# Briimbo/HwBloomRadixJoin

Measured on AMD Instinct MI355X. Metric: probe-tuples/sec, |R|=128M |S|=1024M q=0.01, 1/2/4/8 MI355X; %HBM roofline, higher is better.
Workload: dtype int32

## Files before the change

### hwbloomradixjoin_amd/__init__.py

```python
from __future__ import annotations

import contextlib
import ctypes
import os
from dataclasses import dataclass
from typing import Optional

import numpy as np

__all__ = [
    "BASIC", "BLOCKED", "SECTORIZED", "BloomFilterArgs", "Relation", "Result", "Stats",
    "BPRO", "PRO", "join_materialize_device", "set_materialize", "set_gpus", "BPRH", "BPRHO", "BRJ", "PRH", "PRHO", "RJ", "assert_args", "join_device", "join_device_async", "join_wait", "join_wait_all", "set_async_timing", "generate_device", "generate_device_range",
    "generate_host", "nonunique_threshold", "create_relation_nonunique",
    "create_relation_nonunique_from_pk", "create_relation_fk_from_pk", "create_relation_zipf",
    "rand_stream", "reference_relations", "create_relation_zipf_device",
    "export_filter", "hash_crc", "hash_crapwow", "lib", "LIB_PATH", "shard_range", "write_relation",
]

PKG_DIR = os.path.dirname(os.path.abspath(__file__))
LIB_PATH = os.environ.get("HWBRJ_LIB") or os.path.join(PKG_DIR, "libhwbrj.so")
CLI_PATH = os.path.join(PKG_DIR, "mchashjoins")

BASIC, BLOCKED, SECTORIZED = 0, 1, 2
_VARIANTS = {"basic": BASIC, "blocked": BLOCKED, "sectorized": SECTORIZED}


class _Tuple(ctypes.Structure):
    _fields_ = [("key", ctypes.c_int32), ("payload", ctypes.c_int32)]


class _Relation(ctypes.Structure):
    _fields_ = [("tuples", ctypes.POINTER(_Tuple)), ("num_tuples", ctypes.c_uint64)]


class _Result(ctypes.Structure):
    _fields_ = [("totalresults", ctypes.c_int64), ("resultlist", ctypes.c_void_p),
                ("nthreads", ctypes.c_int)]


class _BloomArgs(ctypes.Structure):
    _fields_ = [("variant", ctypes.c_int), ("m", ctypes.c_uint64), ("k", ctypes.c_uint64),
                ("B", ctypes.c_uint64)]


class _Stats(ctypes.Structure):
    _fields_ = [("filtered", ctypes.c_uint64), ("matches", ctypes.c_int64), ("mode", ctypes.c_int),
                ("format", ctypes.c_int), ("partitions", ctypes.c_uint32),
                ("subparts", ctypes.c_uint32), ("slice_segments", ctypes.c_uint32)] + [
                    (n, ctypes.c_double) for n in (
                        "ms_total", "ms_r_scatter", "ms_r_index", "ms_build", "ms_s_scatter",
                        "ms_s_index", "ms_probe", "ms_surv", "ms_join", "ms_join_probe")] + [
                    ("join_keys", ctypes.c_int), ("unstaged_items", ctypes.c_uint32),
                    ("join_key_bits", ctypes.c_uint32)]

JOIN_KEYS_32, JOIN_KEYS_PACKED, JOIN_KEYS_MIXED = 0, 1, 2


_LIB = None


def lib() -> ctypes.CDLL:
    global _LIB
    if _LIB is None:
        if not os.path.exists(LIB_PATH):
            raise ImportError(f"{LIB_PATH} is missing: run `python -c 'import __graft_entry__ as g; "
                              "g.build()'` (the MI355X HIP library is required; there is no CPU "
                              "fallback)")
        try:
            import torch
        except ImportError:
            pass
        L = ctypes.CDLL(LIB_PATH)
        L.BPRO.restype = ctypes.POINTER(_Result)
        L.BPRO.argtypes = [ctypes.POINTER(_Relation), ctypes.POINTER(_Relation), ctypes.c_int,
                           ctypes.POINTER(_BloomArgs)]
        L.PRO.restype = ctypes.POINTER(_Result)
        L.PRO.argtypes = [ctypes.POINTER(_Relation), ctypes.POINTER(_Relation), ctypes.c_int]
        for nm in ("BPRH", "BPRHO", "BRJ"):
            getattr(L, nm).restype = ctypes.POINTER(_Result)
            getattr(L, nm).argtypes = L.BPRO.argtypes
        for nm in ("PRH", "PRHO", "RJ"):
            getattr(L, nm).restype = ctypes.POINTER(_Result)
            getattr(L, nm).argtypes = L.PRO.argtypes
        L.assert_args.argtypes = [ctypes.POINTER(_BloomArgs)]
        L.hwbrj_join_device.restype = ctypes.c_int
        L.hwbrj_join_device_async.restype = ctypes.c_int
        L.hwbrj_join_device_async.argtypes = [ctypes.c_void_p, ctypes.c_uint64, ctypes.c_void_p,
                                              ctypes.c_uint64, ctypes.c_void_p, ctypes.c_void_p]
        L.hwbrj_join_device_algo.restype = ctypes.c_int
        L.hwbrj_join_device_algo.argtypes = [ctypes.c_void_p, ctypes.c_uint64, ctypes.c_void_p,
                                             ctypes.c_uint64, ctypes.POINTER(_BloomArgs),
                                             ctypes.c_int, ctypes.c_void_p, ctypes.POINTER(_Stats)]
        L.hwbrj_join_wait.restype = ctypes.c_int
        L.hwbrj_join_wait.argtypes = [ctypes.c_void_p]
        L.hwbrj_set_async_timing.restype = ctypes.c_int
        L.hwbrj_set_async_timing.argtypes = [ctypes.c_int]
        L.hwbrj_join_wait_all.restype = ctypes.c_int
        L.hwbrj_join_wait_all.argtypes = [ctypes.c_void_p, ctypes.c_int, ctypes.POINTER(ctypes.c_int)]
        L.hwbrj_join_device.argtypes = [ctypes.c_void_p, ctypes.c_uint64, ctypes.c_void_p,
                                        ctypes.c_uint64, ctypes.POINTER(_BloomArgs),
                                        ctypes.c_void_p, ctypes.POINTER(_Stats)]
        L.hwbrj_join_materialize_device.restype = ctypes.c_int
        L.hwbrj_join_materialize_device.argtypes = [
            ctypes.c_void_p, ctypes.c_uint64, ctypes.c_void_p, ctypes.c_uint64,
            ctypes.POINTER(_BloomArgs), ctypes.c_void_p, ctypes.c_uint64,
            ctypes.POINTER(ctypes.c_uint64), ctypes.c_void_p, ctypes.POINTER(_Stats),
            ctypes.POINTER(ctypes.c_double)]
        L.hwbrj_set_materialize.restype = None
        L.hwbrj_set_materialize.argtypes = [ctypes.c_int]
        L.hwbrj_set_gpus.restype = ctypes.c_int
        L.hwbrj_set_gpus.argtypes = [ctypes.c_int]
        L.hwbrj_generate_device.restype = ctypes.c_int
        L.hwbrj_generate_device.argtypes = [ctypes.c_void_p, ctypes.c_uint64, ctypes.c_uint32,
                                            ctypes.c_uint64, ctypes.c_uint64, ctypes.c_double,
                                            ctypes.c_uint64, ctypes.c_void_p]
        L.hwbrj_generate_device_range.restype = ctypes.c_int
        L.hwbrj_generate_device_range.argtypes = [ctypes.c_void_p, ctypes.c_uint64, ctypes.c_uint64,
                                                  ctypes.c_uint64, ctypes.c_uint32, ctypes.c_uint64,
                                                  ctypes.c_uint64, ctypes.c_double, ctypes.c_uint64,
                                                  ctypes.c_void_p]
        L.hwbrj_generate_host.restype = ctypes.c_int
        L.hwbrj_generate_host.argtypes = [ctypes.c_void_p, ctypes.c_uint64, ctypes.c_uint32,
                                          ctypes.c_uint64, ctypes.c_uint64, ctypes.c_double,
                                          ctypes.c_uint64, ctypes.c_int]
        L.hwbrj_nonunique_threshold.restype = ctypes.c_uint64
        L.hwbrj_nonunique_threshold.argtypes = [ctypes.c_uint64, ctypes.c_double, ctypes.c_int]
        L.hwbrj_create_relation_nonunique.restype = ctypes.c_int
        L.hwbrj_create_relation_nonunique.argtypes = [ctypes.c_void_p, ctypes.c_uint64,
                                                      ctypes.c_int64, ctypes.c_uint32]
        for fn in (L.hwbrj_create_relation_nonunique_from_pk, L.hwbrj_create_relation_fk_from_pk):
            fn.restype = ctypes.c_int
            fn.argtypes = [ctypes.c_void_p, ctypes.c_uint64, ctypes.c_void_p, ctypes.c_uint64,
                           ctypes.c_int64, ctypes.c_double, ctypes.c_uint32]
        L.hwbrj_create_relation_zipf.restype = ctypes.c_int
        L.hwbrj_create_relation_zipf.argtypes = [ctypes.c_void_p, ctypes.c_uint64, ctypes.c_uint64,
                                                 ctypes.c_double, ctypes.c_uint32, ctypes.c_int]
        L.hwbrj_create_relation_zipf_device.restype = ctypes.c_int
        L.hwbrj_create_relation_zipf_device.argtypes = [
            ctypes.c_void_p, ctypes.c_uint64, ctypes.c_uint64, ctypes.c_double, ctypes.c_uint32,
            ctypes.c_double, ctypes.c_int, ctypes.c_void_p]
        L.hwbrj_rand_stream.restype = ctypes.c_int
        L.hwbrj_rand_stream.argtypes = [ctypes.c_uint32, ctypes.c_void_p, ctypes.c_uint64]
        L.hwbrj_write_relation.restype = ctypes.c_int
        L.hwbrj_write_relation.argtypes = [ctypes.POINTER(_Relation), ctypes.c_char_p]
        L.hwbrj_write_result_relation.restype = ctypes.c_int
        L.hwbrj_write_result_relation.argtypes = [ctypes.c_void_p, ctypes.c_char_p]
        L.hwbrj_export_filter.restype = ctypes.c_int
        L.hwbrj_export_filter.argtypes = [ctypes.c_void_p, ctypes.c_uint64]
        L.hwbrj_hash_crc.restype = ctypes.c_uint32
        L.hwbrj_hash_crc.argtypes = [ctypes.c_uint32, ctypes.c_int32]
        L.hwbrj_hash_crapwow.restype = ctypes.c_uint32
        L.hwbrj_hash_crapwow.argtypes = [ctypes.c_uint32, ctypes.c_int32]
        L.hwbrj_device_count.restype = ctypes.c_int
        L.hwbrj_set_device.restype = ctypes.c_int
        L.hwbrj_set_device.argtypes = [ctypes.c_int]
        L.hwbrj_last_error.restype = ctypes.c_char_p
        L.hwbrj_version.restype = ctypes.c_char_p
        L.hwbrj_set_test_hook.restype = ctypes.c_int
        L.hwbrj_set_test_hook.argtypes = [ctypes.c_int, ctypes.c_int64]
        L.hwbrj_tsc_hz.restype = ctypes.c_uint64
        L.hwbrj_copy_bandwidth.restype = ctypes.c_int
        L.hwbrj_copy_bandwidth.argtypes = [ctypes.c_uint64, ctypes.c_int, ctypes.POINTER(ctypes.c_double)]
        L.hwbrj_release.restype = None
        _LIB = L
    return _LIB


def _err(code: int, what: str):
    if code != 0:
        raise RuntimeError(f"{what} failed ({code}): {lib().hwbrj_last_error().decode()}")


@dataclass
class BloomFilterArgs:
    variant: int = BASIC
    m: int = 256 << 20
    k: int = 8
    B: int = 1024

    @classmethod
    def from_flag(cls, b: str, m: int, k: int, B: int = 1024) -> Optional["BloomFilterArgs"]:
        if b == "no":
            return None
        return cls(_VARIANTS.get(b, BASIC), m, k, B)

    def _c(self) -> _BloomArgs:
        return _BloomArgs(int(self.variant), int(self.m), int(self.k), int(self.B))


@dataclass
class Result:
    totalresults: int
    nthreads: int
    pairs: Optional[np.ndarray] = None


class _TupleBuffer(ctypes.Structure):
    pass


_TupleBuffer._fields_ = [("tuples", ctypes.POINTER(_Tuple)), ("next", ctypes.POINTER(_TupleBuffer))]


class _ChainedTupleBuffer(ctypes.Structure):
    _fields_ = [("buf", ctypes.POINTER(_TupleBuffer)), ("readcursor", ctypes.POINTER(_TupleBuffer)),
                ("writecursor", ctypes.POINTER(_TupleBuffer)), ("writepos", ctypes.c_uint32),
                ("readpos", ctypes.c_uint32), ("readlen", ctypes.c_uint32),
                ("numbufs", ctypes.c_uint32)]


class _ThreadResult(ctypes.Structure):
    _fields_ = [("nresults", ctypes.c_int64), ("results", ctypes.c_void_p),
                ("threadid", ctypes.c_uint32)]


_CB_TUPLES = 1024 * 1024


def _take_result(r) -> Result:
    libc = ctypes.CDLL(None)
    res = r.contents
    pairs = None
    if res.resultlist:
        tl = ctypes.cast(res.resultlist, ctypes.POINTER(_ThreadResult))
        parts = []
        for t in range(res.nthreads):
            cb = ctypes.cast(tl[t].results, ctypes.POINTER(_ChainedTupleBuffer)).contents
            n, b, first = tl[t].nresults, cb.buf, True
            while b and n > 0:
                take = min(n, cb.writepos if first else _CB_TUPLES)
                a = np.ctypeslib.as_array(ctypes.cast(b.contents.tuples, ctypes.POINTER(ctypes.c_int32)),
                                          shape=(take * 2,))
                parts.append(a.reshape(-1, 2).copy())
                n -= take
                b, first = b.contents.next, False
            addr = ctypes.cast(cb.buf, ctypes.c_void_p).value
            while addr:
                b = ctypes.cast(addr, ctypes.POINTER(_TupleBuffer)).contents
                nxt = ctypes.cast(b.next, ctypes.c_void_p).value
                libc.free(ctypes.cast(b.tuples, ctypes.c_void_p))
                libc.free(ctypes.c_void_p(addr))
                addr = nxt
            libc.free(ctypes.c_void_p(tl[t].results))
        libc.free(ctypes.cast(res.resultlist, ctypes.c_void_p))
        pairs = np.concatenate(parts) if parts else np.empty((0, 2), dtype=np.int32)
    out = Result(res.totalresults, res.nthreads, pairs)
    libc.free(r)
    return out


HOOK_JOIN_SPLIT, HOOK_PJ_FAIL_RANK, HOOK_BCAST_NONROOT, HOOK_PJ_PLAN_DIV, HOOK_PJ_ASYNC_FAIL = 1, 2, 3, 4, 5
_HOOK_OFF = {HOOK_JOIN_SPLIT: 0, HOOK_PJ_FAIL_RANK: -1, HOOK_BCAST_NONROOT: 0, HOOK_PJ_PLAN_DIV: 0,
             HOOK_PJ_ASYNC_FAIL: 0}


def version() -> str:
    return lib().hwbrj_version().decode()


def set_test_hook(hook: int, value: int) -> None:
    _err(lib().hwbrj_set_test_hook(hook, int(value)), "hwbrj_set_test_hook")


@contextlib.contextmanager
def hooked(hook: int, value: int):
    set_test_hook(hook, value)
    try:
        yield
    finally:
        set_test_hook(hook, _HOOK_OFF[hook])


def set_gpus(gpus: int) -> None:
    _err(lib().hwbrj_set_gpus(int(gpus)), "hwbrj_set_gpus")


def set_materialize(on: bool) -> None:
    lib().hwbrj_set_materialize(1 if on else 0)


@dataclass
class Stats:
    filtered: int
    matches: int
    mode: int
    format: int
    partitions: int
    subparts: int
    slice_segments: int
    ms_total: float
    ms_r_scatter: float
    ms_r_index: float
    ms_build: float
    ms_s_scatter: float
    ms_s_index: float
    ms_probe: float
    ms_surv: float
    ms_join: float
    ms_join_probe: float
    join_keys: int = 0
    unstaged_items: int = 0
    join_key_bits: int = 32


class Relation:

    def __init__(self, tuples: np.ndarray):
        t = np.ascontiguousarray(tuples, dtype=np.int32)
        if t.ndim != 2 or t.shape[1] != 2:
            raise ValueError("tuples must have shape (N, 2): key, payload")
        self.tuples = t
        self._c = _Relation(t.ctypes.data_as(ctypes.POINTER(_Tuple)), t.shape[0])

    @property
    def num_tuples(self) -> int:
        return self.tuples.shape[0]


def write_relation(rel: "Relation | np.ndarray", filename: str) -> None:
    r = rel if isinstance(rel, Relation) else Relation(rel)
    _err(lib().hwbrj_write_relation(ctypes.byref(r._c), os.fsencode(filename)), "hwbrj_write_relation")


def assert_args(args: BloomFilterArgs) -> bool:
    m, B = int(args.m), int(args.B)
    if m & (m - 1):
        return False
    if args.variant != BASIC and (B <= 0 or B & (B - 1) or m % B):
        return False
    return True


def BPRO(relR: Relation, relS: Relation, nthreads: int, args: BloomFilterArgs) -> Result:
    a = args._c()
    return _take_result(lib().BPRO(ctypes.byref(relR._c), ctypes.byref(relS._c), int(nthreads),
                                   ctypes.byref(a)))


def PRO(relR: Relation, relS: Relation, nthreads: int) -> Result:
    return _take_result(lib().PRO(ctypes.byref(relR._c), ctypes.byref(relS._c), int(nthreads)))


def _run(name: str, relR: Relation, relS: Relation, nthreads: int, args=None) -> Result:
    fn = getattr(lib(), name)
    r = (fn(ctypes.byref(relR._c), ctypes.byref(relS._c), int(nthreads), ctypes.byref(args._c()))
         if args is not None else fn(ctypes.byref(relR._c), ctypes.byref(relS._c), int(nthreads)))
    return _take_result(r)


def BPRH(relR, relS, nthreads, args):
    return _run("BPRH", relR, relS, nthreads, args)


def BPRHO(relR, relS, nthreads, args):
    return _run("BPRHO", relR, relS, nthreads, args)


def BRJ(relR, relS, nthreads, args):
    return _run("BRJ", relR, relS, nthreads, args)


def PRH(relR, relS, nthreads):
    return _run("PRH", relR, relS, nthreads)


def PRHO(relR, relS, nthreads):
    return _run("PRHO", relR, relS, nthreads)


def RJ(relR, relS, nthreads):
    return _run("RJ", relR, relS, nthreads)


def _ptr(t) -> int:
    return int(t.data_ptr())


def _check_rel(R, S):
    import torch
    for name, t in (("R", R), ("S", S)):
        if (not t.is_cuda or t.dtype != torch.int32 or t.dim() != 2 or t.shape[1] != 2
                or not t.is_contiguous()):
            raise ValueError(f"{name} must be a contiguous (N, 2) torch.int32 tensor on the GPU")
    if R.device != S.device:
        raise ValueError(f"R is on {R.device} but S is on {S.device}")
    _err(lib().hwbrj_set_device(R.device.index or 0), "hwbrj_set_device")


def join_device_async(R, S, args: Optional[BloomFilterArgs] = None, stream=None) -> None:
    _check_rel(R, S)
    a = args._c() if args is not None else None
    sp = ctypes.c_void_p(stream.cuda_stream) if stream is not None else None
    _err(lib().hwbrj_join_device_async(_ptr(R), R.shape[0], _ptr(S), S.shape[0],
                                       ctypes.byref(a) if a is not None else None, sp),
         "hwbrj_join_device_async")


def join_wait() -> Stats:
    st = _Stats()
    _err(lib().hwbrj_join_wait(ctypes.byref(st)), "hwbrj_join_wait")
    return Stats(**{n: getattr(st, n) for n, _ in _Stats._fields_})


def set_async_timing(on: bool) -> None:
    _err(lib().hwbrj_set_async_timing(1 if on else 0), "hwbrj_set_async_timing")


def join_wait_all(capacity: int = 256) -> list:
    arr = (_Stats * max(1, capacity))()
    n = ctypes.c_int(0)
    _err(lib().hwbrj_join_wait_all(arr, capacity, ctypes.byref(n)), "hwbrj_join_wait_all")
    return [Stats(**{f: getattr(arr[i], f) for f, _ in _Stats._fields_}) for i in range(n.value)]


ALGO_PRO, ALGO_PRH, ALGO_PRHO = 0, 1, 2


def join_device(R, S, args: Optional[BloomFilterArgs] = None, stream=None,
                algorithm: int = ALGO_PRO) -> Stats:
    _check_rel(R, S)
    st = _Stats()
    a = args._c() if args is not None else None
    sp = ctypes.c_void_p(stream.cuda_stream) if stream is not None else None
# ... 142 lines not shown
```

### hwbloomradixjoin_amd/csrc/hwbrj_api.cpp

```cpp
#include <stdio.h>
#include <stdlib.h>
#include <string.h>
#include <x86intrin.h>

#include <algorithm>
#include <chrono>
#include <mutex>
#include <set>
#include <string>
#include <thread>
#include <vector>

#include "hwbrj_engine.h"

namespace hwbrj {

static thread_local std::string g_last_error;
void set_last_error(const std::string& s) { g_last_error = s; }

}

using namespace hwbrj;

extern "C" {

const char* hwbrj_last_error(void) { return g_last_error.c_str(); }
#ifndef HWBRJ_SRC_SHA
#define HWBRJ_SRC_SHA "dev"
#endif
const char* hwbrj_version(void) {
    static const std::string base = [] {
        std::string k = kernel_build_knobs();
        const std::string d = dev_knobs_string();
        if (!d.empty()) k += (k.empty() ? "" : " ") + d;
        return k;
    }();
    static std::mutex            mu;
    static std::set<std::string> interned;
    std::lock_guard<std::mutex>  lk(mu);
    std::string        k = base;
    const TestHooks&   h = test_hooks();
    auto add = [&](const std::string& w) { k += (k.empty() ? "" : " ") + w; };
    if (h.join_split) add("HWBRJ_HOOK_JOIN_SPLIT=" + std::to_string(h.join_split));
    if (h.pj_fail_rank >= 0) add("HWBRJ_HOOK_PJ_FAIL_RANK=" + std::to_string(h.pj_fail_rank));
    if (h.bcast_nonroot) add("HWBRJ_HOOK_BCAST_NONROOT=" + std::to_string(h.bcast_nonroot));
    if (h.pj_plan_div) add("HWBRJ_HOOK_PJ_PLAN_DIV=" + std::to_string(h.pj_plan_div));
    if (h.pj_async_fail) add("HWBRJ_HOOK_PJ_ASYNC_FAIL=" + std::to_string(h.pj_async_fail));
    const std::string v = std::string("hwbloomradixjoin_amd 0.6 (gfx950) src " HWBRJ_SRC_SHA) +
                          (k.empty() ? "" : " knobs: " + k);
    return interned.insert(v).first->c_str();
}

int hwbrj_set_test_hook(int hook, int64_t value) {
    TestHooks& h = test_hooks();
    switch (hook) {
        case HWBRJ_HOOK_JOIN_SPLIT:
            if (value < 0 || value > 0xFFFFFFFFll) break;
            h.join_split = (uint32_t) value;
            return 0;
        case HWBRJ_HOOK_PJ_FAIL_RANK:
            h.pj_fail_rank = (int) value;
            return 0;
        case HWBRJ_HOOK_BCAST_NONROOT:
            if (value < 0 || value > 2) break;
            h.bcast_nonroot = (int) value;
            return 0;
        case HWBRJ_HOOK_PJ_PLAN_DIV:
            if (value < 0 || value > 1000000) break;
            h.pj_plan_div = (int) value;
            return 0;
        case HWBRJ_HOOK_PJ_ASYNC_FAIL:
            if (value < 0 || value > 1) break;
            h.pj_async_fail = (int) value;
            return 0;
        default:
            set_last_error("unknown test hook");
            return 2;
    }
    set_last_error("test hook value out of range");
    return 2;
}

int hwbrj_device_count(void) {
    int n = 0;
    if (hipGetDeviceCount(&n) != hipSuccess) return 0;
    return n;
}

int hwbrj_set_device(int device) {
    hipError_t e = hipSetDevice(device);
    if (e != hipSuccess) {
        set_last_error(std::string("hipSetDevice: ") + hipGetErrorString(e));
        return 1;
    }
    return 0;
}

void hwbrj_release(void) {
    Engine* e = engine_for_current_device();
    if (e) e->release();
}

uint64_t hwbrj_tsc_hz(void) {
    static const uint64_t hz = [] {
        const auto     t0 = std::chrono::steady_clock::now();
        const uint64_t c0 = __rdtsc();
        std::this_thread::sleep_for(std::chrono::milliseconds(50));
        const uint64_t c1 = __rdtsc();
        const double   s  = std::chrono::duration<double>(std::chrono::steady_clock::now() - t0).count();
        return (uint64_t) ((double) (c1 - c0) / s);
    }();
    return hz;
}

int hwbrj_copy_bandwidth(uint64_t bytes, int reps, double* gbps) {
    if (!gbps || reps < 1 || bytes < 16 || bytes % 16) {
        set_last_error("hwbrj_copy_bandwidth: bytes must be a positive multiple of 16, reps >= 1");
        return 1;
    }
    void *a = nullptr, *b = nullptr;
    if (hipMalloc(&a, bytes) != hipSuccess || hipMalloc(&b, bytes) != hipSuccess) {
        if (a) (void) hipFree(a);
        set_last_error("hwbrj_copy_bandwidth: hipMalloc failed");
        return 6;
    }
    hipStream_t st = nullptr;
    hipEvent_t  e0 = nullptr, e1 = nullptr;
    int         rc = 0;
    std::vector<float> ms;
    if (hipStreamCreateWithFlags(&st, hipStreamNonBlocking) != hipSuccess || hipEventCreate(&e0) != hipSuccess ||
        hipEventCreate(&e1) != hipSuccess || hipMemsetAsync(a, 1, bytes, st) != hipSuccess) {
        rc = 3;
    } else {
        int dev = 0, cus = 256;
        (void) hipGetDevice(&dev);
        (void) hipDeviceGetAttribute(&cus, hipDeviceAttributeMultiprocessorCount, dev);
        launch_copy_bw(a, b, bytes, cus, st);
        for (int r = 0; r < reps && rc == 0; r++) {
            float t = 0;
            (void) hipEventRecord(e0, st);
            launch_copy_bw(a, b, bytes, cus, st);
            (void) hipEventRecord(e1, st);
            if (hipEventSynchronize(e1) != hipSuccess || hipEventElapsedTime(&t, e0, e1) != hipSuccess) rc = 3;
            ms.push_back(t);
        }
    }
    if (rc == 0) {
        std::sort(ms.begin(), ms.end());
        *gbps = 2.0 * (double) bytes / (ms[ms.size() / 2] * 1e-3) / 1e9;
    } else {
        set_last_error(std::string("hwbrj_copy_bandwidth: ") + hipGetErrorString(hipGetLastError()));
    }
    if (e0) (void) hipEventDestroy(e0);
    if (e1) (void) hipEventDestroy(e1);
    if (st) (void) hipStreamDestroy(st);
    (void) hipFree(a);
    (void) hipFree(b);
    return rc;
}

uint32_t hwbrj_hash_crc(uint32_t seed, int32_t key) { return crc_f_bitwise(seed ^ (uint32_t) key); }
uint32_t hwbrj_hash_crapwow(uint32_t seed, int32_t key) { return crapwow(seed, (uint32_t) key); }

int hwbrj_join_device(const tuple_t* d_R, uint64_t nR, const tuple_t* d_S, uint64_t nS,
                      const bloom_filter_args_t* args, void* stream, hwbrj_stats_t* stats) {
    Engine* e = engine_for_current_device();
    if (!e) return 10;
    return e->run((const uint2*) d_R, nR, (const uint2*) d_S, nS, args, (hipStream_t) stream, stats);
}

int hwbrj_join_device_algo(const tuple_t* d_R, uint64_t nR, const tuple_t* d_S, uint64_t nS,
                           const bloom_filter_args_t* args, int algorithm, void* stream,
                           hwbrj_stats_t* stats) {
    Engine* e = engine_for_current_device();
    if (!e) return 10;
    return e->run((const uint2*) d_R, nR, (const uint2*) d_S, nS, args, (hipStream_t) stream, stats, algorithm);
}

int hwbrj_join_device_async(const tuple_t* d_R, uint64_t nR, const tuple_t* d_S, uint64_t nS,
                            const bloom_filter_args_t* args, void* stream) {
    Engine* e = engine_for_current_device();
    if (!e) return 10;
    return e->run_async((const uint2*) d_R, nR, (const uint2*) d_S, nS, args, (hipStream_t) stream);
}

int hwbrj_join_partitioned(const hwbrj_exchange_t* x, int rank, int world, const tuple_t* d_R,
                           uint64_t nR, uint64_t nR_total, const tuple_t* d_S, uint64_t nS,
                           const bloom_filter_args_t* args, hwbrj_stats_t* stats) {
    if (!x || !x->buffer || !x->alltoall_u64 || !x->alltoallv || !x->allgather) {
        set_last_error("incomplete exchange (hwbrj_exchange_t)");
        return 2;
    }
    Engine* e = engine_for_current_device();
    if (!e) return 10;
    return e->join_partitioned(x, rank, world, (const uint2*) d_R, nR, nR_total, (const uint2*) d_S, nS,
                               args, stats);
}

int hwbrj_join_wait(hwbrj_stats_t* stats) {
    Engine* e = engine_for_current_device();
    if (!e) return 10;
    return e->wait(stats);
}

int hwbrj_set_async_timing(int on) {
    Engine* e = engine_for_current_device();
    if (!e) return 10;
    e->set_async_timing(on != 0);
    return 0;
}

int hwbrj_join_wait_all(hwbrj_stats_t* stats, int capacity, int* n_joins) {
    if (capacity < 0 || (capacity > 0 && !stats)) {
        set_last_error("stats must hold capacity >= 0 entries");
        return 2;
    }
    Engine* e = engine_for_current_device();
    if (!e) return 10;
    return e->wait_all(stats, capacity, n_joins);
}

static int materialize_pairs(Engine* e, const tuple_t* d_R, uint64_t nR, const tuple_t* d_S, uint64_t nS,
                             const bloom_filter_args_t* args, tuple_t* d_out, uint64_t cap, uint64_t* n,
                             hipStream_t stream, hwbrj_stats_t* st, double* ms) {
    int rc = e->run_mat((const uint2*) d_R, nR, (const uint2*) d_S, nS, args, stream,
                        MatReq{(uint2*) d_out, cap}, st);
    if (rc == 0) {
        *n = (uint64_t) st->matches;
        if (ms) *ms = st->ms_total;
        return 0;
    }
    if (rc != kRcMatGlobal) return rc;
    rc = e->run((const uint2*) d_R, nR, (const uint2*) d_S, nS, args, stream, st);
// ... 445 lines not shown
```

### hwbloomradixjoin_amd/csrc/hwbrj_engine.cpp

```cpp
#include "hwbrj_engine.h"

#include <stdio.h>
#include <stdlib.h>
#include <string.h>

#include <algorithm>
#include <mutex>
#include <vector>

namespace hwbrj {

#define HWBRJ_CHECK(expr)                                                                 \
    do {                                                                                  \
        hipError_t e_ = (expr);                                                           \
        if (e_ != hipSuccess) {                                                           \
            set_last_error(std::string(#expr) + ": " + hipGetErrorString(e_));            \
            return 1;                                                                     \
        }                                                                                 \
    } while (0)

bool build_crc_tables(CrcTables* t) {
    uint32_t col[32];
    for (int i = 0; i < 32; i++) col[i] = crc_f_bitwise(1u << i);
    for (int j = 0; j < 8; j++)
// ... 113 lines not shown
            g->B          = (uint32_t) B;
            g->nblocks    = (uint32_t) std::min<uint64_t>(m / B, 0xFFFFFFFFull);
            g->block_span = (uint32_t) ((B / 8) * 8);
        }
        uint64_t F = 0;
        if (a->variant == BASIC) {
            if (k >= 1 && m >= 32 && k * nR <= (1ull << 31)) {
                g->mode = MODE_SLICE_BASIC;
                F       = std::min<uint64_t>(1024, m / 32);
            } else {
                g->mode = MODE_GLOBAL;
            }
        } else {
            if (B >= 8 && m >= 32 && (m / B) <= 0xFFFFFFFFull) {
                g->mode = MODE_SLICE_BLOCK;
                F       = std::min<uint64_t>(std::min<uint64_t>(1024, m / B), m / 32);
                if (dev_knobs().maxf) F = std::min<uint64_t>(F, dev_knobs().maxf);
            } else {
                g->mode = MODE_GLOBAL;
            }
        }
        g->log2F = (g->mode == MODE_GLOBAL) ? kMaxLog2F : ilog2u(F);
        if (g->mode == MODE_SLICE_BLOCK || g->mode == MODE_SLICE_BASIC) {
            g->slice_bits = (uint32_t) (m >> g->log2F);
            g->seg_bits   = std::min(g->slice_bits, kSliceMaxBits);
            g->nseg       = g->slice_bits / g->seg_bits;
            g->seg_words  = std::max<uint32_t>(4, g->seg_bits / 32);
        }
        if (g->mode == MODE_SLICE_BLOCK && ilog2u(B) <= g->log2F) g->format = FMT_PACKED;
        g->s_format = g->format;
        if (g->mode == MODE_SLICE_BLOCK || g->mode == MODE_SLICE_BASIC) g->log2seg = ilog2u(g->seg_bits);
        if (a->variant != BASIC) {
            g->log2B    = ilog2u(B);
            g->log2secw = std::min<uint32_t>(g->log2B, 6);
            g->nsecmask = (uint32_t) (B >> g->log2secw) - 1u;
            if (g->mode == MODE_SLICE_BLOCK) g->lbmask = (g->nblocks >> g->log2F) - 1u;
        }
    }
    const uint64_t F    = 1ull << g->log2F;
    const uint64_t rper = (nR + F - 1) / F;
    uint32_t       l2s  = 0;
    g->sub_shift  = (g->mode == MODE_SLICE_BASIC) ? 0 : g->log2F;
    if (mat && g->sub_shift > 0) {
        l2s = g->log2F >= 15 ? 0 : std::min<uint32_t>(6, 15 - g->log2F);
        while (l2s < 6 && (rper >> l2s) > 4000) l2s++;
    } else if (mat) {
        while (l2s < 6 && (rper >> l2s) > 1536) l2s++;
    } else if (g->sub_shift > 0 && g->log2F + 6 >= 14) {
        l2s = g->log2F >= 14 ? 0 : 14 - g->log2F;
        if (dev_knobs().l2sub && g->log2F + dev_knobs().l2sub >= 14)
            l2s = std::min<uint32_t>(6, dev_knobs().l2sub);
    } else {
        while (l2s < 6 && (rper >> l2s) > 4096) l2s++;
    }
    if (g->sub_shift + l2s == 0) l2s = 1;
    g->log2NSUB   = l2s;
    g->hash_shift = g->sub_shift + g->log2NSUB;
    return true;
}

bool DevBuf::ensure(size_t need) {
    if (need == 0) need = 16;
    if (need <= bytes) return true;
    release();
    if (hipMalloc(&p, need) != hipSuccess) {
        p     = nullptr;
        bytes = 0;
        return false;
    }
    bytes = need;
    return true;
}

void DevBuf::release() {
    if (p) (void) hipFree(p);
    p     = nullptr;
    bytes = 0;
}

const DevKnobs& dev_knobs() {
    static const DevKnobs k = [] {
        DevKnobs d;
#ifdef HWBRJ_DEV_BUILD
        auto u = [](const char* n) -> uint32_t {
            const char* e = getenv(n);
            return e ? (uint32_t) strtoul(e, nullptr, 0) : 0u;
        };
        d.kk1       = getenv("HWBRJ_DEV_KK1") != nullptr;
        d.kk_gather = getenv("HWBRJ_DEV_KK_GATHER") != nullptr;
        d.noxcd     = getenv("HWBRJ_DEV_NOXCD") != nullptr;
        d.dbg       = getenv("HWBRJ_DBG") != nullptr;
        d.maxf      = u("HWBRJ_DEV_MAXF");
        d.scwpc     = u("HWBRJ_DEV_SCWPC");
        if (getenv("HWBRJ_DEV_EVFLAGS")) d.evflags = (int) u("HWBRJ_DEV_EVFLAGS");
        d.l2sub     = u("HWBRJ_DEV_L2SUB");
        d.ovl       = getenv("HWBRJ_DEV_OVL") != nullptr;
        d.rfirst    = getenv("HWBRJ_DEV_RFIRST") != nullptr;
#endif
        return d;
    }();
    return k;
}

std::string dev_knobs_string() {
    const DevKnobs& d = dev_knobs();
    std::string     r;
    auto add = [&](const std::string& w) { r += (r.empty() ? "" : " ") + w; };
    if (d.kk1) add("HWBRJ_DEV_KK1");
    if (d.kk_gather) add("HWBRJ_DEV_KK_GATHER");
    if (d.noxcd) add("HWBRJ_DEV_NOXCD");
    if (d.dbg) add("HWBRJ_DBG");
    if (d.maxf) add("HWBRJ_DEV_MAXF=" + std::to_string(d.maxf));
    if (d.scwpc) add("HWBRJ_DEV_SCWPC=" + std::to_string(d.scwpc));
    if (d.evflags >= 0) add("HWBRJ_DEV_EVFLAGS=" + std::to_string(d.evflags));
    if (d.l2sub) add("HWBRJ_DEV_L2SUB=" + std::to_string(d.l2sub));
    if (d.ovl) add("HWBRJ_DEV_OVL");
    if (d.rfirst) add("HWBRJ_DEV_RFIRST");
    return r;
}

TestHooks& test_hooks() {
    static TestHooks h;
    return h;
}

Engine::Engine(int device) : device_(device) {
    (void) dev_knobs();
    (void) hipSetDevice(device);
    hipDeviceProp_t prop;
    if (hipGetDeviceProperties(&prop, device) == hipSuccess) cus_ = prop.multiProcessorCount;
    (void) hipStreamCreateWithFlags(&own_stream_, hipStreamNonBlocking);
    const unsigned evf = dev_knobs().evflags >= 0 ? (unsigned) dev_knobs().evflags : hipEventDisableSystemFence;
    for (int i = 0; i < 10; i++)
        (void) (i < 8 ? hipEventCreateWithFlags(&ev_[i], evf) : hipEventCreate(&ev_[i]));
    CrcTables t;
    if (!build_crc_tables(&t)) set_last_error("CRC table inversion failed");
    (void) hipMalloc((void**) &d_tabs_, sizeof(CrcTables));
    (void) hipMemcpy(d_tabs_, &t, sizeof(CrcTables), hipMemcpyHostToDevice);
    (void) hipMalloc((void**) &d_plan_, sizeof(GenPlan));
}

Engine::~Engine() { release(); }

void Engine::release() {
    (void) pj_drain();
    pj_q_.clear();
    if (pj_plan_.valid) pj_lost_ = true;
    for (DevBuf* b : {&pjX, &pjRitems, &pjRing}) b->release();
    for (DevBuf* b : {&poolR, &metaR, &usedR, &wgqcR, &wgqeR, &wgqoR, &lstartR, &estartR, &istartR,
                      &listR, &poolS, &metaS, &usedS, &wgqcS, &wgqeS, &wgqoS, &lstartS, &estartS,
                      &istartS, &listS, &slices, &bitmap, &rjoin, &rrun, &surv, &survcnt, &survoff,
                      &dense, &small, &bpos, &colR, &colS, &mtab, &mcount, &jtask, &jparts, &pjList,
                      &pjLstart, &pjSweep, &pjTab, &pjRegion, &pjTot, &pjSoff, &pjIbase, &pjCnt, &pjOff,
                      &pjIstart, &pjJobs, &ppoolR, &ppoolS, &rpay, &survpos, &dense2, &kkcnt, &xcnt_, &pjBsum, &pjBound, &pjWtot, &pjWscan, &pjTab2})
        b->release();
    for (DevBuf& b : xslot_) b.release();
    if (pending_) (void) hipEventSynchronize(ev_[8]);
    ring_drop();
    jring_.release();
    have_filter_ = false;
}

static size_t ring_slot_bytes() { return 128 + join_sum_slots() * join_sum_stride() * 8; }

static uint64_t region_cap(uint64_t n, uint32_t G, uint32_t F) {
    const uint64_t units = (n + 3) / 4;
    const uint64_t per   = ((units + G - 1) / G) * 4;
    return (per + 31) / 32 + F + 1;
}

int Engine::run(const uint2* dR, uint64_t nR, const uint2* dS, uint64_t nS,
                const bloom_filter_args_t* args, hipStream_t stream, hwbrj_stats_t* st, int jkind) {
    const int rc = enqueue(dR, nR, dS, nS, args, stream, dev_knobs().dbg, jkind);
    return rc ? rc : wait(st);
}

int Engine::run_async(const uint2* dR, uint64_t nR, const uint2* dS, uint64_t nS,
                      const bloom_filter_args_t* args, hipStream_t stream, int jkind) {
    phase_ev_    = false;
    const int rc = enqueue(dR, nR, dS, nS, args, stream, false, jkind);
    phase_ev_    = true;
    return rc;
}

hipError_t Engine::mark(int i, hipStream_t stream) {
    return phase_ev_ ? hipEventRecord(ev_[i], stream) : hipSuccess;
}

int Engine::reserve(const uint2* dR, uint64_t nR, const uint2* dS, uint64_t nS,
                    const bloom_filter_args_t* args, int jkind) {
    alloc_only_  = true;
    const int rc = enqueue(dR, nR, dS, nS, args, nullptr, false, jkind);
    alloc_only_  = false;
    last_nj_     = 0;
    return rc;
}

int Engine::run_mat(const uint2* dR, uint64_t nR, const uint2* dS, uint64_t nS,
                    const bloom_filter_args_t* args, hipStream_t stream, const MatReq& mat,
                    hwbrj_stats_t* st) {
    const int rc = enqueue(dR, nR, dS, nS, args, stream, false, 0, &mat);
    return rc ? rc : wait(st);
}

int Engine::enqueue(const uint2* dR, uint64_t nR, const uint2* dS, uint64_t nS,
                    const bloom_filter_args_t* args, hipStream_t stream, bool dbg, int jkind,
                    const MatReq* mat) {
    if (jkind < 0 || jkind > 2) {
        set_last_error("unknown per-partition join algorithm");
        return 2;
    }
    HWBRJ_CHECK(hipSetDevice(device_));
    Geometry    g;
    std::string err;
    if (!plan_geometry(args, nR, &g, &err, mat != nullptr)) {
        set_last_error(err);
        return 2;
    }
    if (mat && g.mode == MODE_GLOBAL) {
        set_last_error("global-bitmap mode: materialized by the side pass");
        return kRcMatGlobal;
    }
    const bool kk1 = dev_knobs().kk1;
    if (!mat && g.mode == MODE_SLICE_BASIC && (g.k > 1 || kk1) && (uint64_t) g.k * nR <= (1ull << 31) &&
        !dev_knobs().kk_gather) {
        if (!stream) stream = own_stream_;
        if (pending_ && stream != pending_stream_) HWBRJ_CHECK(hipStreamWaitEvent(stream, ev_[8], 0));
        return enqueue_basic_kk(dR, nR, dS, nS, g, stream, jkind);
    }
    if (!stream) stream = own_stream_;
    if (pending_ && stream != pending_stream_) HWBRJ_CHECK(hipStreamWaitEvent(stream, ev_[8], 0));
    const uint32_t F = 1u << g.log2F, NSUB = 1u << g.log2NSUB, NJ = F * NSUB;
    const bool     slice_mode = g.mode == MODE_SLICE_BLOCK || g.mode == MODE_SLICE_BASIC;
    const uint32_t nseg       = slice_mode ? g.nseg : 1;
    const uint32_t CH         = probe_chunks_per_item();
    const size_t   sc_lds     = mat ? scatter_pay_lds_bytes(g.log2F) : scatter_lds_bytes(g.log2F);
    uint32_t       sc_wpc     = (uint32_t) std::max<size_t>(1, std::min<size_t>(2, 163840 / sc_lds));
    if (dev_knobs().scwpc)
        sc_wpc = std::max(1u, std::min(sc_wpc, dev_knobs().scwpc));
    const uint32_t G          = (uint32_t) cus_ * sc_wpc;
    const bool     basic_kk = g.mode == MODE_SLICE_BASIC && g.k > 1;
    const uint64_t nRk      = basic_kk ? (uint64_t) g.k * nR : 0;
    const bool bcast = bcast_ && comm_ && slice_mode && !basic_kk;
    auto pre = [&](int rc) -> int {
        if (!bcast || alloc_only_) return rc;
        return rccl_agree_status(comm_, comm_world_, comm_rank_, rc, stream, &agree_);
    };
    const uint64_t capR = region_cap(nR, G, F), capS = region_cap(std::max(nS, nRk), G, F);
    const uint64_t LR = (uint64_t) G * capR, LS = (uint64_t) G * capS;
    const uint64_t items_max = (LS / CH + F + 1) * nseg;
    if (G > 512) {
        set_last_error("more than 512 scatter workgroups (k_plan row groups)");
        return pre(3);
    }
    if (LS > (1ull << 27) || LR > (1ull << 27) || capS >= (1u << 22) || capR >= (1u << 22)) {
        set_last_error("relation too large for 27-bit chunk ids (|S| or |R| > ~4.2e9 tuples per GPU)");
        return pre(3);
    }
    if (mat && (capS >= (1u << 21) || capR >= (1u << 21))) {
        set_last_error("relation too large for the materializing scatter's 22-bit half indices");
        return pre(3);
    }
    const uint64_t GF = (uint64_t) G * F;
    bool ok = true;
    ok &= poolR.ensure(LR * 128) && metaR.ensure(LR * 2) && listR.ensure(LR * 4);
    ok &= usedR.ensure(G * 4) && wgqcR.ensure(GF * 4) && wgqeR.ensure(GF * 4) && wgqoR.ensure(GF * 4);
    ok &= lstartR.ensure((F + 1) * 4) && estartR.ensure((F + 1) * 8) && istartR.ensure((F + 1) * 4);
    ok &= poolS.ensure(LS * 128) && metaS.ensure(LS * 2) && listS.ensure(LS * 4);
    ok &= usedS.ensure(G * 4) && wgqcS.ensure(GF * 4) && wgqeS.ensure(GF * 4) && wgqoS.ensure(GF * 4);
    ok &= lstartS.ensure((F + 1) * 4) && estartS.ensure((F + 1) * 8) && istartS.ensure((F + 1) * 4);
    const uint64_t BSW = build_chunks_per_sweep(), SLOT = build_sweep_slot();
    const uint64_t sweeps_max = LR / BSW + F + 1;
    ok &= rjoin.ensure(sweeps_max * SLOT * 4) && rrun.ensure(2 * sweeps_max * NSUB * 4);
    ok &= surv.ensure(nseg * LS * 128) && survcnt.ensure(items_max * NSUB * 4) &&
          survoff.ensure(items_max * NSUB * 4);
    ok &= jring_.ensure(kJoinRing * ring_slot_bytes()) && colR.ensure(F * 12) && colS.ensure(F * 12);
    const bool jnew = jparts.bytes < (size_t) (2 * NJ + 1) * 4 || NJ != last_nj_;
    last_nj_ = NJ;
    ok &= jtask.ensure((size_t) join_extra_tasks() * 8) && jparts.ensure((size_t) (2 * NJ + 1) * 4);
    if (slice_mode) ok &= slices.ensure((uint64_t) F * nseg * g.seg_words * 4);
    if (g.mode == MODE_GLOBAL) ok &= bitmap.ensure(((g.m + 31) / 32) * 4) && dense.ensure(nS * 4);
    if (basic_kk) ok &= bpos.ensure(nRk * 4);
    if (mat) {
        ok &= ppoolR.ensure(LR * 128) && ppoolS.ensure(LS * 128) && rpay.ensure(sweeps_max * SLOT * 4) &&
              survpos.ensure(nseg * LS * 128);
    }
    if (!ok) {
        set_last_error("hipMalloc failed (device memory)");
        return pre(4);
    }
    if (alloc_only_) return 0;
    if (const int rc = pre(0)) return rc;
    uint32_t  rslot      = 0;
    bool      rtimed     = false;
    char*     sm         = (char*) ring_take(&rslot);
    if (!sm) return 1;
    uint64_t* d_result   = (uint64_t*) sm;
    uint64_t* d_dcount   = (uint64_t*) sm + 1;
    uint64_t* d_filtered = (uint64_t*) sm + 2;

    if (jnew) HWBRJ_CHECK(hipMemsetAsync(jparts.p, 0, jparts.bytes, stream));
    if (g.mode == MODE_GLOBAL) HWBRJ_CHECK(hipMemsetAsync(bitmap.p, 0, bitmap.bytes, stream));

    ScatterParams sp{};
    sp.tabs = d_tabs_;
    sp.g    = g;
    sp.zero_small = (uint32_t*) sm;
    sp.zero_word  = jparts.as<uint32_t>() + 2 * NJ;

    auto s_pass = [&](hipStream_t st, bool marks, hipEvent_t* tev = nullptr) -> int {
        ScatterParams ss = sp;
        ss.zero_small    = nullptr;
        ss.zero_word     = nullptr;
        if (g.mode == MODE_GLOBAL) {
            launch_probe_global(dS, nS, g, d_tabs_, bitmap.as<uint32_t>(), dense.as<uint32_t>(),
                                d_dcount, st);
            ss.src   = dense.p;
            ss.n     = nS;
            ss.n_dev = d_dcount;
        } else {
            ss.src   = dS;
            ss.n     = nS;
            ss.n_dev = nullptr;
        }
        ss.pool       = poolS.as<uint32_t>();
        ss.meta       = metaS.as<uint32_t>();
        ss.wg_used    = usedS.as<uint32_t>();
        ss.wgq_chunks = wgqcS.as<uint32_t>();
        ss.wgq_elems  = wgqeS.as<uint32_t>();
        ss.cap        = capS;
        if (dbg) {
            if (!dbgS.ensure((size_t) G * 64)) {
                set_last_error("hipMalloc failed (device memory)");
                return 4;
            }
            HWBRJ_CHECK(hipMemsetAsync(dbgS.p, 0, dbgS.bytes, st));
            ss.dbg = dbgS.as<uint64_t>();
        }
        ss.ppool = mat ? ppoolS.as<uint32_t>() : nullptr;
        if (tev) HWBRJ_CHECK(hipEventRecord(tev[0], st));
        launch_scatter(ss, g.mode == MODE_GLOBAL ? SRC_CODES : SRC_TUPLES, SIDE_S, G, st);
        if (tev) HWBRJ_CHECK(hipEventRecord(tev[1], st));
        if (marks) HWBRJ_CHECK(mark(4, st));
        launch_plan(wgqcS.as<uint32_t>(), wgqeS.as<uint32_t>(), G, g.log2F, wgqoS.as<uint32_t>(),
                    colS.as<uint32_t>() + 2 * F, colS.as<uint64_t>(), st);
        launch_list_fill(metaS.as<uint32_t>(), usedS.as<uint32_t>(), capS, g.log2F, wgqoS.as<uint32_t>(),
                         colS.as<uint32_t>() + 2 * F, colS.as<uint64_t>(), CH, nseg, lstartS.as<uint32_t>(),
                         estartS.as<uint64_t>(), istartS.as<uint32_t>(), listS.as<uint32_t>(), G, st);
        if (marks) HWBRJ_CHECK(mark(5, st));
        return 0;
    };
    HWBRJ_CHECK(mark(0, stream));
    const bool ovl = (dev_knobs().ovl || (HWBRJ_OVL_ASYNC && !phase_ev_)) && g.mode != MODE_GLOBAL && !basic_kk &&
                     !mat && !bcast;
    if (ovl) {
        if (!ovl_stream_) {
            HWBRJ_CHECK(hipStreamCreateWithFlags(&ovl_stream_, hipStreamNonBlocking));
            HWBRJ_CHECK(hipEventCreateWithFlags(&ovl_ev_[0], hipEventDisableTiming));
            HWBRJ_CHECK(hipEventCreateWithFlags(&ovl_ev_[1], hipEventDisableTiming));
        }
        HWBRJ_CHECK(hipEventRecord(ovl_ev_[0], stream));
        HWBRJ_CHECK(hipStreamWaitEvent(ovl_stream_, ovl_ev_[0], 0));
        hipEvent_t* tev = nullptr;
        if (async_timing_) {
            for (int i = 0; i < 2; i++)
                if (!tev_[rslot][i]) HWBRJ_CHECK(hipEventCreateWithFlags(&tev_[rslot][i], hipEventDisableSystemFence));
            tev = tev_[rslot];
        }
        rtimed = tev != nullptr;
        if (const int rc = s_pass(ovl_stream_, false, tev)) return rc;
        HWBRJ_CHECK(hipEventRecord(ovl_ev_[1], ovl_stream_));
    }
    const bool s_first = !ovl && !dev_knobs().rfirst && g.mode != MODE_GLOBAL && !basic_kk;
    if (s_first)
        if (const int rc = s_pass(stream, true)) return rc;
    if (g.mode == MODE_GLOBAL)
        launch_build_global(dR, nR, g, d_tabs_, bitmap.as<uint32_t>(), stream);
    sp.src        = dR;
    sp.n          = nR;
    sp.n_dev      = nullptr;
    sp.pool       = poolR.as<uint32_t>();
    sp.ppool      = mat ? ppoolR.as<uint32_t>() : nullptr;
    sp.meta       = metaR.as<uint32_t>();
    sp.wg_used    = usedR.as<uint32_t>();
    sp.wgq_chunks = wgqcR.as<uint32_t>();
    sp.wgq_elems  = wgqeR.as<uint32_t>();
    sp.cap        = capR;
    launch_scatter(sp, SRC_TUPLES, SIDE_R, G, stream);
    HWBRJ_CHECK(mark(1, stream));
    launch_plan(wgqcR.as<uint32_t>(), wgqeR.as<uint32_t>(), G, g.log2F, wgqoR.as<uint32_t>(),
                colR.as<uint32_t>() + 2 * F, colR.as<uint64_t>(), stream);
    launch_list_fill(metaR.as<uint32_t>(), usedR.as<uint32_t>(), capR, g.log2F, wgqoR.as<uint32_t>(),
                     colR.as<uint32_t>() + 2 * F, colR.as<uint64_t>(), (uint32_t) BSW, 1, lstartR.as<uint32_t>(),
                     estartR.as<uint64_t>(), istartR.as<uint32_t>(), listR.as<uint32_t>(), G, stream);
    HWBRJ_CHECK(mark(2, stream));
    sp.ppool      = nullptr;
    sp.zero_small = nullptr;
    sp.zero_word  = nullptr;
    BuildParams bp{};
    bp.g          = g;
    bp.tabs       = d_tabs_;
    bp.pool       = poolR.as<uint32_t>();
    bp.list       = listR.as<uint32_t>();
    bp.list_start = lstartR.as<uint32_t>();
    bp.elem_start = estartR.as<uint64_t>();
    bp.slices     = slice_mode ? slices.as<uint32_t>() : nullptr;
    bp.sweep_start = istartR.as<uint32_t>();
    bp.out_codes   = rjoin.as<uint32_t>();
    bp.run_cnt     = rrun.as<uint32_t>();
    bp.run_off     = rrun.as<uint32_t>() + sweeps_max * NSUB;
    bp.ppool       = mat ? ppoolR.as<uint32_t>() : nullptr;
    bp.out_pay     = mat ? rpay.as<uint32_t>() : nullptr;
    const bool     pack3 = !mat && join_pack3(g) && pack3_hint_;
    const uint32_t kbits = pack3 ? join_key_bits(g) : 0u;
    bp.kbits       = kbits;
    const int nonroot_hook = bcast && comm_world_ == 1 ? test_hooks().bcast_nonroot : 0;
    bp.no_slices = bcast && (comm_rank_ != 0 || nonroot_hook) ? 1u : 0u;
    if (nonroot_hook == 2) HWBRJ_CHECK(hipMemsetAsync(slices.p, 0, slices.bytes, stream));
    launch_build(bp, F, stream);
    if (bcast) {
        const int rc = rccl_broadcast(comm_, slices.p, (size_t) F * nseg * g.seg_words * 4, 0, stream);
        if (rc) {
            (void) hipEventRecord(ev_[8], stream);
            pending_        = true;
            pending_stream_ = stream;
            pending_rc_     = rc;
            pending_err_    = hwbrj_last_error();
            return rc;
        }
    }
    if (basic_kk) {
        launch_bitpos(dR, nR, g, bpos.as<uint32_t>(), stream);
        sp.src        = bpos.p;
        sp.n          = nRk;
        sp.n_dev      = nullptr;
        sp.pool       = poolS.as<uint32_t>();
        sp.meta       = metaS.as<uint32_t>();
        sp.wg_used    = usedS.as<uint32_t>();
        sp.wgq_chunks = wgqcS.as<uint32_t>();
        sp.wgq_elems  = wgqeS.as<uint32_t>();
        sp.cap        = capS;
        launch_scatter(sp, SRC_CODES, SIDE_R, G, stream);
        launch_plan(wgqcS.as<uint32_t>(), wgqeS.as<uint32_t>(), G, g.log2F, wgqoS.as<uint32_t>(),
                    colS.as<uint32_t>() + 2 * F, colS.as<uint64_t>(), stream);
        launch_list_fill(metaS.as<uint32_t>(), usedS.as<uint32_t>(), capS, g.log2F, wgqoS.as<uint32_t>(),
                         colS.as<uint32_t>() + 2 * F, colS.as<uint64_t>(), (uint32_t) BSW, 1,
                         lstartS.as<uint32_t>(), estartS.as<uint64_t>(), istartS.as<uint32_t>(),
                         listS.as<uint32_t>(), G, stream);
        launch_slice_fill(poolS.as<uint32_t>(), listS.as<uint32_t>(), lstartS.as<uint32_t>(), g,
                          slices.as<uint32_t>(), stream);
    }
    HWBRJ_CHECK(mark(3, stream));
    if (ovl) {
        HWBRJ_CHECK(hipStreamWaitEvent(stream, ovl_ev_[1], 0));
        HWBRJ_CHECK(mark(4, stream));
        HWBRJ_CHECK(mark(5, stream));
    } else if (!s_first) {
        if (const int rc = s_pass(stream, true)) return rc;
    }
    ProbeParams pp{};
    pp.g               = g;
    pp.tabs            = d_tabs_;
    pp.pool            = poolS.as<uint32_t>();
    pp.list            = listS.as<uint32_t>();
    pp.list_start      = lstartS.as<uint32_t>();
    pp.item_start      = istartS.as<uint32_t>();
    pp.slices          = slice_mode ? slices.as<uint32_t>() : nullptr;
    pp.surv            = surv.as<uint32_t>();
    pp.surv_seg_stride = LS * 32;
    pp.surv_cnt        = survcnt.as<uint32_t>();
    pp.surv_off        = survoff.as<uint32_t>();
    pp.filtered        = d_filtered;
    pp.job_surv        = jparts.as<uint32_t>() + NJ;
    pp.surv_pos        = mat ? survpos.as<uint32_t>() : nullptr;
    pp.kbits           = kbits;
    pp.fmt_cnt         = mat ? nullptr : (uint32_t*) sm + 10;
    const size_t   pl_lds = probe_lds_bytes(g, nullptr, mat != nullptr);
    const uint32_t PG = (uint32_t) cus_ * (uint32_t) std::max<size_t>(1, std::min<size_t>(2, 163840 / pl_lds));
    const bool dbg_on = dbg;
    if (dbg_on) {
        ok &= dbgP.ensure((size_t) std::max<uint32_t>(PG, F) * 64) && dbgJ.ensure((size_t) std::max<uint64_t>(F, 1024) * 64);
        HWBRJ_CHECK(hipMemsetAsync(dbgP.p, 0, dbgP.bytes, stream));
        HWBRJ_CHECK(hipMemsetAsync(dbgJ.p, 0, dbgJ.bytes, stream));
        pp.dbg = dbgP.as<uint64_t>();
    }
    launch_probe(pp, PG, stream);
    HWBRJ_CHECK(mark(6, stream));
    surv_fused_ = true;
    JoinParams jp{};
    jp.r_codes         = rjoin.as<uint32_t>();
    jp.r_sweep_start   = istartR.as<uint32_t>();
    jp.r_cnt           = rrun.as<uint32_t>();
    jp.r_off           = rrun.as<uint32_t>() + sweeps_max * NSUB;
    jp.slot            = (uint32_t) SLOT;
    jp.surv            = surv.as<uint32_t>();
    jp.surv_cnt        = survcnt.as<uint32_t>();
    jp.surv_off        = survoff.as<uint32_t>();
    jp.item_start      = istartS.as<uint32_t>();
    jp.list_start      = lstartS.as<uint32_t>();
    jp.surv_seg_stride = LS * 32;
    jp.nseg            = nseg;
    jp.CH              = CH;
    jp.log2NSUB        = g.log2NSUB;
    jp.hash_shift      = g.hash_shift;
    jp.bitmap          = (g.sub_shift > 0 && 32 - g.hash_shift <= join_bitmap_log2()) ? 1u : 0u;
    jp.jsum            = (uint64_t*) (sm + 128);
    jp.dbg             = dbg_on ? dbgJ.as<uint64_t>() : nullptr;
    jp.nparts          = jparts.as<uint32_t>();
    jp.extra           = jtask.as<uint2>();
    jp.nextra          = jparts.as<uint32_t>() + 2 * NJ;
    jp.jkind           = (uint32_t) jkind;
    jp.split_surv      = test_hooks().join_split;
    jp.r_kbits         = kbits;
    jp.fmt_cnt         = pp.fmt_cnt;
    jp.timing          = phase_ev_ ? 1u : 0u;
    if (mat) {
        HWBRJ_CHECK(hipMemsetAsync(jparts.as<uint32_t>() + NJ, 0, (size_t) NJ * 4, stream));
        MatJoinParams mp{};
        mp.r_codes         = jp.r_codes;
        mp.r_pay           = rpay.as<uint32_t>();
        mp.r_sweep_start   = jp.r_sweep_start;
        mp.r_cnt           = jp.r_cnt;
        mp.r_off           = jp.r_off;
        mp.slot            = jp.slot;
        mp.surv            = jp.surv;
        mp.surv_pos        = survpos.as<uint32_t>();
        mp.surv_cnt        = jp.surv_cnt;
        mp.surv_off        = jp.surv_off;
        mp.item_start      = jp.item_start;
        mp.list_start      = jp.list_start;
        mp.surv_seg_stride = jp.surv_seg_stride;
        mp.nseg            = nseg;
        mp.CH              = CH;
        mp.log2NSUB        = g.log2NSUB;
        mp.hash_shift      = g.hash_shift;
        mp.bm              = (g.sub_shift > 0 && 32 - g.hash_shift <= 17) ? 1u : 0u;
        mp.s_pay           = ppoolS.as<uint32_t>();
        mp.out             = mat->out;
        mp.cap             = mat->cap;
        mp.count           = (unsigned long long*) d_result;
        launch_join_mat(mp, NJ, stream);
    } else {
        launch_join(jp, NJ, jparts.as<uint32_t>() + NJ, stream);
    }
    HWBRJ_CHECK(hipEventRecord(ev_[8], stream));
    HWBRJ_CHECK(hipGetLastError());
    pending_      = true;
    pending_rc_   = 0;
    pending_args_ = args != nullptr;
    pending_nS_   = nS;
    pending_ev_   = phase_ev_;
    pending_sfirst_ = s_first;
    pending_fmt_    = pp.fmt_cnt != nullptr;
    pending_slots_  = !mat;
    pending_stream_ = stream;
    have_filter_  = args != nullptr;
    last_g_       = g;
    {
        JoinRec r;
        r.slot  = rslot;
        r.args  = args != nullptr;
        r.fmt   = pending_fmt_;
        r.kbits = kbits;
        r.slots = !mat;
        r.timed = rtimed;
        r.nS    = nS;
        r.g     = g;
        ring_push(r);
    }

    if (dbg_on) {
        HWBRJ_CHECK(hipEventSynchronize(ev_[8]));
        std::vector<uint64_t> hp(PG * 8);
        HWBRJ_CHECK(hipMemcpy(hp.data(), dbgP.p, hp.size() * 8, hipMemcpyDeviceToHost));
        double sp_[6] = {0};
        for (uint32_t b = 0; b < PG; b++)
            for (int k = 0; k < 6; k++) sp_[k] += (double) hp[b * 8 + k] / PG;
        std::vector<uint64_t> hs(G * 8);
        HWBRJ_CHECK(hipMemcpy(hs.data(), dbgS.p, hs.size() * 8, hipMemcpyDeviceToHost));
        double ss[6] = {0};
        for (uint32_t b = 0; b < G; b++)
            for (int k = 0; k < 6; k++) ss[k] += (double) hs[b * 8 + k] / G;
        fprintf(stderr, "[dbg] S scatter cyc/WG: hash %.0f load+flush %.0f rank %.0f b1 %.0f write+plan %.0f b2 %.0f\n",
                ss[0], ss[1], ss[2], ss[3], ss[4], ss[5]);
        {
            uint64_t t0 = ~0ull;
            std::vector<double> st(G), en(G);
            for (uint32_t b = 0; b < G; b++) t0 = std::min<uint64_t>(t0, hs[b * 8 + 6]);
            for (uint32_t b = 0; b < G; b++) {
                st[b] = (hs[b * 8 + 6] - t0) / 100.0;
                en[b] = (hs[b * 8 + 7] - t0) / 100.0;
            }
            std::sort(st.begin(), st.end());
            std::sort(en.begin(), en.end());
            fprintf(stderr, "[dbg] S scatter WG start us: max %.1f | end us: min %.1f p10 %.1f p50 %.1f p90 %.1f max %.1f\n",
                    st[G - 1], en[0], en[G / 10], en[G / 2], en[G * 9 / 10], en[G - 1]);
        }
        fprintf(stderr, "[dbg] probe cyc/WG: top %.0f test %.0f b1 %.0f scan+b2 %.0f write %.0f b3+copy %.0f\n",
                sp_[0], sp_[1], sp_[2], sp_[3], sp_[4], sp_[5]);
        {
            std::vector<uint64_t> hj2(1024 * 8);
            HWBRJ_CHECK(hipMemcpy(hj2.data(), dbgJ.p, hj2.size() * 8, hipMemcpyDeviceToHost));
            double sj2[6] = {0};
            const double nwg = (double) F * (1u << g.log2NSUB);
            for (uint32_t b = 0; b < 1024; b++)
                for (int k = 0; k < 6; k++) sj2[k] += (double) hj2[b * 8 + k] / nwg;
            fprintf(stderr, "[dbg] join cyc/WG (wave 0): desc %.0f R+sets %.0f popcnt %.0f surv1 %.0f surv2 %.0f end %.0f\n",
                    sj2[0], sj2[1], sj2[2], sj2[3], sj2[4], sj2[5]);
        }
    }
    return 0;
}

int Engine::enqueue_basic_kk(const uint2* dR, uint64_t nR, const uint2* dS, uint64_t nS,
                             const Geometry& g, hipStream_t stream, int jkind) {
    Geometry    gj;
    std::string err;
    if (!plan_geometry(nullptr, nR, &gj, &err)) {
        set_last_error(err);
        return 2;
    }
    const uint32_t F = 1u << g.log2F, Fj = 1u << gj.log2F, Fm = std::max(F, Fj);
    const uint32_t NSUB = 1u << gj.log2NSUB, NJ = Fj * NSUB;
    const uint32_t nseg = g.nseg, CH = probe_chunks_per_item();
    const uint32_t G    = (uint32_t) cus_;
    const uint64_t nRk  = (uint64_t) g.k * nR;
    const uint64_t Ib   = ((nS / 32 + (uint64_t) G * (Fm + 1)) / CH + Fm + 1) * nseg;
    const uint64_t rw   = ((Ib + G - 1) / G) * CH * 32;
    const uint64_t capR = region_cap(nR, G, Fm);
    const uint64_t capS = std::max(region_cap(std::max(nS, nRk), G, Fm), rw / 32 + Fm + 1);
    const uint64_t LR = (uint64_t) G * capR, LS = (uint64_t) G * capS;
    const uint64_t items_max = (LS / CH + Fm + 1) * nseg;
    if (G > 512 || LS > (1ull << 27) || LR > (1ull << 27) || capS >= (1u << 22) || capR >= (1u << 22)) {
        set_last_error("relation too large for 27-bit chunk ids (|S| or |R| > ~4.2e9 tuples per GPU)");
        return 3;
    }
    const uint64_t GF = (uint64_t) G * Fm;
    bool ok = true;
    ok &= poolR.ensure(LR * 128) && metaR.ensure(LR * 2) && listR.ensure(LR * 4);
    ok &= usedR.ensure(G * 4) && wgqcR.ensure(GF * 4) && wgqeR.ensure(GF * 4) && wgqoR.ensure(GF * 4);
    ok &= lstartR.ensure((Fm + 1) * 4) && estartR.ensure((Fm + 1) * 8) && istartR.ensure((Fm + 1) * 4);
    ok &= poolS.ensure(LS * 128) && metaS.ensure(LS * 2) && listS.ensure(LS * 4);
    ok &= usedS.ensure(G * 4) && wgqcS.ensure(GF * 4) && wgqeS.ensure(GF * 4) && wgqoS.ensure(GF * 4);
    ok &= lstartS.ensure((Fm + 1) * 4) && estartS.ensure((Fm + 1) * 8) && istartS.ensure((Fm + 1) * 4);
    const uint64_t BSW = build_chunks_per_sweep(), SLOT = build_sweep_slot();
    const uint64_t sweeps_max = LR / BSW + Fm + 1;
    ok &= rjoin.ensure(sweeps_max * SLOT * 4) && rrun.ensure(2 * sweeps_max * NSUB * 4);
    ok &= surv.ensure(LS * 128) && survcnt.ensure(items_max * NSUB * 4) && survoff.ensure(items_max * NSUB * 4);
    ok &= jring_.ensure(kJoinRing * ring_slot_bytes()) && colR.ensure(Fm * 12) && colS.ensure(Fm * 12);
    const bool jnew = jparts.bytes < (size_t) (2 * NJ + 1) * 4 || NJ != last_nj_;
    last_nj_ = NJ;
    ok &= jtask.ensure((size_t) join_extra_tasks() * 8) && jparts.ensure((size_t) (2 * NJ + 1) * 4);
    ok &= slices.ensure((uint64_t) F * nseg * g.seg_words * 4) && (g.k <= G || bpos.ensure(nRk * 4));
    const uint32_t NC = (g.k + 64) & ~63u;
    ok &= dense.ensure(G * rw * 4) && dense2.ensure(G * rw * 4) && kkcnt.ensure(NC * 8 + 2 * G * 4);
    if (!ok) {
        set_last_error("hipMalloc failed (device memory)");
        return 4;
    }
    if (alloc_only_) return 0;
    uint32_t  rslot      = 0;
    char*     sm         = (char*) ring_take(&rslot);
    if (!sm) return 1;
    uint64_t* d_filtered = (uint64_t*) sm + 2;
    uint64_t* cnt        = kkcnt.as<uint64_t>();
    uint32_t* wgc[2]     = {(uint32_t*) (cnt + NC), (uint32_t*) (cnt + NC) + G};
    HWBRJ_CHECK(hipMemsetAsync(sm, 0, 64, stream));
    HWBRJ_CHECK(hipMemsetAsync(kkcnt.p, 0, kkcnt.bytes, stream));
    if (jnew) HWBRJ_CHECK(hipMemsetAsync(jparts.p, 0, jparts.bytes, stream));
    HWBRJ_CHECK(hipMemsetAsync(jparts.as<uint32_t>() + 2 * NJ, 0, 4, stream));

    auto side = [&](bool r) {
        ScatterParams sp{};
        sp.tabs       = d_tabs_;
        sp.pool       = (r ? poolR : poolS).as<uint32_t>();
        sp.meta       = (r ? metaR : metaS).as<uint32_t>();
        sp.wg_used    = (r ? usedR : usedS).as<uint32_t>();
        sp.wgq_chunks = (r ? wgqcR : wgqcS).as<uint32_t>();
        sp.wgq_elems  = (r ? wgqeR : wgqeS).as<uint32_t>();
        sp.cap        = r ? capR : capS;
        return sp;
    };
    auto index = [&](bool r, uint32_t log2F, uint32_t ch, uint32_t ns) {
        const uint32_t Fx = 1u << log2F;
        DevBuf& col = r ? colR : colS;
        launch_plan((r ? wgqcR : wgqcS).as<uint32_t>(), (r ? wgqeR : wgqeS).as<uint32_t>(), G, log2F,
                    (r ? wgqoR : wgqoS).as<uint32_t>(), col.as<uint32_t>() + 2 * Fx, col.as<uint64_t>(), stream);
        launch_list_fill((r ? metaR : metaS).as<uint32_t>(), (r ? usedR : usedS).as<uint32_t>(), r ? capR : capS,
                         log2F, (r ? wgqoR : wgqoS).as<uint32_t>(), col.as<uint32_t>() + 2 * Fx, col.as<uint64_t>(),
                         ch, ns, (r ? lstartR : lstartS).as<uint32_t>(), (r ? estartR : estartS).as<uint64_t>(),
                         (r ? istartR : istartS).as<uint32_t>(), (r ? listR : listS).as<uint32_t>(), G, stream);
    };

    HWBRJ_CHECK(mark(0, stream));
    ScatterParams sp = side(true);
    sp.g   = gj;
    sp.src = dR;
    sp.n   = nR;
    launch_scatter(sp, SRC_TUPLES, SIDE_R, G, stream);
    HWBRJ_CHECK(mark(1, stream));
    index(true, gj.log2F, (uint32_t) BSW, 1);
    HWBRJ_CHECK(mark(2, stream));
    BuildParams bp{};
    bp.g           = gj;
    bp.tabs        = d_tabs_;
    bp.pool        = poolR.as<uint32_t>();
    bp.list        = listR.as<uint32_t>();
    bp.list_start  = lstartR.as<uint32_t>();
    bp.elem_start  = estartR.as<uint64_t>();
    bp.sweep_start = istartR.as<uint32_t>();
    bp.out_codes   = rjoin.as<uint32_t>();
    bp.run_cnt     = rrun.as<uint32_t>();
    bp.run_off     = rrun.as<uint32_t>() + sweeps_max * NSUB;
    launch_build(bp, Fj, stream);
    sp = side(false);
    if (g.k <= G) {
        Geometry gp = g;
        gp.mode     = MODE_BASIC_POS;
        sp.g        = gp;
        sp.src      = dR;
        sp.n        = nRk;
        sp.vn       = nR;
        launch_scatter(sp, SRC_TUPLES, SIDE_R, G, stream);
    } else {
        launch_bitpos(dR, nR, g, bpos.as<uint32_t>(), stream);
        sp.g   = g;
        sp.src = bpos.p;
        sp.n   = nRk;
        launch_scatter(sp, SRC_CODES, SIDE_R, G, stream);
    }
    index(false, g.log2F, (uint32_t) BSW, 1);
    launch_slice_fill(poolS.as<uint32_t>(), listS.as<uint32_t>(), lstartS.as<uint32_t>(), g,
                      slices.as<uint32_t>(), stream);
    HWBRJ_CHECK(mark(3, stream));
    sp     = side(false);
    sp.g   = g;
    sp.src = dS;
    sp.n   = nS;
    launch_scatter(sp, SRC_TUPLES, SIDE_S, G, stream);
    HWBRJ_CHECK(mark(4, stream));
    index(false, g.log2F, CH, nseg);
    HWBRJ_CHECK(mark(5, stream));
    const uint32_t PG = G;
    ProbeParams    pb{};
    pb.pool       = poolS.as<uint32_t>();
    pb.list       = listS.as<uint32_t>();
    pb.list_start = lstartS.as<uint32_t>();
    pb.item_start = istartS.as<uint32_t>();
    pb.slices     = slices.as<uint32_t>();
    uint32_t* dz[2] = {dense.as<uint32_t>(), dense2.as<uint32_t>()};
// ... 357 lines not shown
```

### hwbloomradixjoin_amd/csrc/hwbrj_engine.h

```cpp
#pragma once

#include <hip/hip_runtime.h>
#include <stdint.h>

#include <deque>
#include <string>
#include <vector>

#include "../../include/hwbrj.h"
#include "hwbrj_common.h"
#include "hwbrj_kernels.h"

namespace hwbrj {

bool plan_geometry(const bloom_filter_args_t* args, uint64_t nR, Geometry* g, std::string* err,
                   bool mat = false);

struct MatReq {
    uint2*   out;
    uint64_t cap;
};
constexpr int kRcMatGlobal = 11;

struct DevBuf {
// ... 18 lines not shown
    void set_async_timing(bool on) { async_timing_ = on; }
    int  reserve(const uint2* dR, uint64_t nR, const uint2* dS, uint64_t nS,
                 const bloom_filter_args_t* args, int jkind = 0);
    int  export_filter(uint8_t* host_out, uint64_t nbytes);
    int  run_mat(const uint2* dR, uint64_t nR, const uint2* dS, uint64_t nS,
                 const bloom_filter_args_t* args, hipStream_t stream, const MatReq& mat,
                 hwbrj_stats_t* st);
    int  materialize(const uint2* dR, uint64_t nR, const uint2* dS, uint64_t nS, uint2* out,
                     uint64_t cap, uint64_t* n, hipStream_t stream, double* ms);
    int  generate(uint2* d_out, uint64_t n, uint64_t offset, uint64_t count, uint32_t nthreads,
                  uint64_t maxid, uint64_t threshold, double selectivity, uint64_t seed,
                  hipStream_t stream);
    int  join_partitioned(const hwbrj_exchange_t* x, int rank, int world, const uint2* dR,
                          uint64_t nR, uint64_t nR_total, const uint2* dS, uint64_t nS,
                          const bloom_filter_args_t* args, hwbrj_stats_t* st, bool native = false);
    void release();
    int  device() const { return device_; }

    int  comm_init(const uint8_t* unique_id, int world, int rank);
    int  comm_destroy();
    bool has_comm() const { return comm_ != nullptr; }
    int  comm_world() const { return comm_world_; }
    int  comm_rank() const { return comm_rank_; }
    int  join_partitioned_rccl(const uint2* dR, uint64_t nR, uint64_t nR_total, const uint2* dS,
                               uint64_t nS, const bloom_filter_args_t* args, hwbrj_stats_t* st);
    void set_filter_broadcast(bool on) { bcast_ = on; }
    hipStream_t stream() const { return own_stream_; }
    DevBuf*     xslot(int s) { return &xslot_[s]; }
    DevBuf*     xcnt() { return &xcnt_; }
    void*       comm() const { return comm_; }
    hwbrj_exchange_t native_exchange();

    static constexpr int kPjDepth = 8;
    static constexpr int kPjKey   = 10;
    int  join_partitioned_async(const hwbrj_exchange_t* x, int rank, int world, const uint2* dR, uint64_t nR,
                                uint64_t nR_total, const uint2* dS, uint64_t nS, const bloom_filter_args_t* args);
    int  join_partitioned_wait(hwbrj_stats_t* st);
    void pj_async_info(uint64_t* out) const;
    bool pj_make_plan() const { return pj_make_plan_; }
    int  pj_plan_from_sync(int world, int rank, uint64_t nR, uint64_t nR_total, uint64_t nS,
                           const bloom_filter_args_t* args, uint64_t mr, uint64_t mi, uint64_t mw);
    int  pj_drain();

  private:
    struct PjGeom {
        Geometry g{};
        uint32_t F = 0, NSUB = 0, W = 0, QL = 0, q0 = 0, nseg = 1, CH = 0, G = 0, NC = 0, items_max = 0;
        uint64_t BSW = 0, SLOT = 0, capR = 0, capS = 0, LS = 0;
        bool     slice_mode = false;
    };
    struct PjPlan {
        bool     valid = false;
        uint64_t BR = 0, BI = 0, BW = 0;
        uint64_t key[kPjKey] = {};
    };
    struct PjX {
        hwbrj_exchange_t x{};
        bool             native = true;
        int              rank = 0, world = 1;
    };
    struct PjIn {
        PjX                 xc;
        const uint2*        dR = nullptr;
        const uint2*        dS = nullptr;
        uint64_t            nR = 0, nR_total = 0, nS = 0;
        bool                has_args = false;
        bloom_filter_args_t args{};
    };
    struct PjPending {
        PjIn          in;
        PjGeom        G;
        bool          sync = false;
        bool          failed_mode = false;
        int           rc   = 0;
        int           slot = 0;
        hwbrj_stats_t st{};
    };
    bool pj_geom(int world, int rank, uint64_t nR, uint64_t nR_total, uint64_t nS,
                 const bloom_filter_args_t* args, PjGeom* G);
    int  pj_async_alloc(const PjGeom& G, const PjPlan& p, bool all, const PjX& c);
    int  pj_a2a_u64(const PjX& c, const uint64_t* d_send, uint64_t* d_recv, uint64_t n);
    int  pj_max_dev(const PjX& c, uint64_t* d, uint64_t n);
    int  pj_max_host(const PjX& c, uint64_t* h, uint64_t n);
    int  pj_establish_plan(const PjGeom& G, uint64_t mr, uint64_t mi, uint64_t mw, const uint64_t* key);
    int  pj_sync_join(const PjIn& in, hwbrj_stats_t* st);
    PjPlan                pj_plan_;
    PjX                   pj_cur_;
    bloom_filter_args_t   pj_plan_args_{};
    bool                  pj_make_plan_ = false;
    bool                  pj_lost_      = false;
    std::deque<PjPending> pj_q_;
    uint64_t              pj_seq_ = 0, pj_async_ = 0, pj_sync_ = 0, pj_fallbacks_ = 0, pj_plans_ = 0;
    uint64_t              pj_last_flag_ = 0, pj_last_sizes_[3] = {0, 0, 0};
    DevBuf                pjX, pjRitems, pjRing;
    hipEvent_t            pjEv_[2 * kPjDepth] = {};

  private:
    void*        comm_       = nullptr;
    int          comm_world_ = 1, comm_rank_ = 0;
    bool         bcast_      = false;
    DevBuf       xslot_[HWBRJ_PJ_NSLOTS], xcnt_;
    DevBuf       agree_;
    int          device_;
    int          cus_ = 256;
    hipStream_t  own_stream_ = nullptr;
    hipStream_t  ovl_stream_ = nullptr;
    hipEvent_t   ovl_ev_[2]  = {nullptr, nullptr};
    hipEvent_t   ev_[10];
    bool         have_filter_ = false;
    Geometry     last_g_{};
    bool         pending_      = false;
    bool         pending_args_ = false;
    uint64_t     pending_nS_   = 0;
    uint32_t     last_nj_      = 0;
    bool         phase_ev_     = true;
    bool         pending_ev_   = true;
    hipStream_t  pending_stream_ = nullptr;
    bool         pending_sfirst_ = false;
    bool         pending_fmt_    = false;
    bool         pending_slots_  = false;
    bool         pack3_hint_     = true;
    int          pending_rc_     = 0;
    std::string  pending_err_;
    bool         surv_fused_   = false;
    struct JoinRec {
        uint32_t slot = 0;
        bool     args = false, fmt = false, slots = false, timed = false;
        uint32_t kbits = 0;
        uint64_t nS   = 0;
        Geometry g{};
    };
    DevBuf                     jring_;
    std::vector<JoinRec>       jr_;
    std::vector<hwbrj_stats_t> jdone_;
    uint32_t                   jr_next_ = 0;
    hwbrj_stats_t              last_st_{};
    bool                       async_timing_ = false;
    hipEvent_t                 tev_[kJoinRing][2] = {};
    void*        ring_take(uint32_t* slot);
    void         ring_push(const JoinRec& r) { jr_.push_back(r); }
    int          ring_collect();
    void         ring_drop() { jr_.clear(); jdone_.clear(); }
    hipError_t   mark(int i, hipStream_t stream);
    bool         alloc_only_   = false;
    int          enqueue(const uint2* dR, uint64_t nR, const uint2* dS, uint64_t nS,
                         const bloom_filter_args_t* args, hipStream_t stream, bool dbg, int jkind,
                         const MatReq* mat = nullptr);
    int          enqueue_basic_kk(const uint2* dR, uint64_t nR, const uint2* dS, uint64_t nS,
                                  const Geometry& g, hipStream_t stream, int jkind);
    CrcTables*   d_tabs_ = nullptr;
    GenPlan*     d_plan_ = nullptr;
    DevBuf poolR, metaR, usedR, wgqcR, wgqeR, wgqoR, lstartR, estartR, istartR, listR;
    DevBuf poolS, metaS, usedS, wgqcS, wgqeS, wgqoS, lstartS, estartS, istartS, listS;
    DevBuf slices, bitmap, rjoin, rrun, surv, survcnt, survoff, dense, small, dbgP, dbgJ, dbgS;
    DevBuf bpos;
    DevBuf colR, colS;
    DevBuf mtab, mcount;
    DevBuf ppoolR, ppoolS, rpay, survpos;
    DevBuf dense2, kkcnt;
    DevBuf jtask, jparts;
    DevBuf pjList, pjLstart, pjSweep, pjTab, pjRegion, pjTot, pjSoff, pjIbase, pjCnt, pjOff, pjIstart, pjJobs;
    DevBuf pjBsum, pjBound, pjWtot, pjWscan, pjTab2;
};

Engine* engine_for_current_device();
void    set_last_error(const std::string& s);

int rccl_broadcast(void* comm, void* buf, size_t bytes, int root, hipStream_t stream);
int read_join_counts(const void* small, bool slots, hipStream_t stream, uint64_t h[6]);
int rccl_agree_status(void* comm, int world, int rank, int rc, hipStream_t stream, DevBuf* tmp);
class Engine;
int rccl_alltoall_u64_dev(Engine* e, const uint64_t* d_send, uint64_t* d_recv, uint64_t n);
int rccl_allreduce_max_u64(Engine* e, uint64_t* d, uint64_t n);
bool rccl_self_blocks();
uint64_t pj_region_cap(uint64_t n, uint32_t G, uint32_t F);

struct GlibcRand {
    int32_t st[31];
    int     f = 3, r = 0;
    void    seed(uint32_t s);
    int32_t next() {
        st[f]           = (int32_t) ((uint32_t) st[f] + (uint32_t) st[r]);
        const int32_t v = (int32_t) ((uint32_t) st[f] >> 1);
        f               = f == 30 ? 0 : f + 1;
        r               = r == 30 ? 0 : r + 1;
        return v;
    }
};

}
```

### hwbloomradixjoin_amd/csrc/hwbrj_kernels.h

```cpp
#pragma once

#include <hip/hip_runtime.h>

#include <string>
#include <stddef.h>
#include <stdint.h>

#include "hwbrj_common.h"

namespace hwbrj {

enum Source : int { SRC_TUPLES = 0, SRC_CODES = 1 };

struct ScatterParams {
    const void*      src;
    uint64_t         n;
    const uint64_t*  n_dev;
    uint32_t*        pool;
    uint32_t*        ppool;
    uint32_t*        meta;
    uint32_t*        wg_used;
    uint32_t*        wgq_chunks;
    uint32_t*        wgq_elems;
    uint64_t*        dbg;
    uint64_t         cap;
    const uint32_t*  seg_cnt;
    uint64_t         seg_stride;
    uint64_t         vn;
    uint32_t*        zero_small;
    uint32_t*        zero_word;
    Geometry         g;
    const CrcTables* tabs;
};

#ifndef HWBRJ_PACK3
#define HWBRJ_PACK3 1
#endif
#ifndef HWBRJ_PACK18
#define HWBRJ_PACK18 1
#endif
inline bool join_pack3(const Geometry& g) { return HWBRJ_PACK3 != 0 && g.sub_shift > 0 && g.hash_shift >= 8; }
inline uint32_t join_key_bits(const Geometry& g) {
    return !join_pack3(g) ? 0u : (HWBRJ_PACK18 && g.hash_shift == 14) ? 18u : 24u;
}

#ifndef HWBRJ_OVL_ASYNC
#define HWBRJ_OVL_ASYNC 1
#endif
#ifndef HWBRJ_PJ_OVL
#define HWBRJ_PJ_OVL 1
#endif

struct BuildParams {
    Geometry         g;
    const CrcTables* tabs;
    const uint32_t*  pool;
    const uint32_t*  list;
    const uint32_t*  list_start;
    const uint64_t*  elem_start;
    uint32_t*        slices;
    const uint32_t*  sweep_start;
    uint32_t*        out_codes;
    uint32_t*        run_cnt;
    uint32_t*        run_off;
    uint32_t         q_base;
    const uint32_t*  ppool;
    uint32_t*        out_pay;
    uint32_t         no_slices;
    uint32_t         kbits;
};

struct ProbeParams {
    Geometry         g;
    const CrcTables* tabs;
    const uint32_t*  pool;
    const uint32_t*  list;
    const uint32_t*  list_start;
    const uint32_t*  item_start;
    const uint32_t*  slices;
    uint32_t*        surv;
    uint64_t         surv_seg_stride;
    uint32_t*        surv_cnt;
    uint32_t*        surv_off;
    uint64_t*        filtered;
    uint32_t*        job_surv;
    uint32_t         stage_cap;
    uint32_t*        surv_pos;
    uint32_t*        wg_cnt;
    uint64_t*        dbg;
    uint32_t         kbits;
    uint32_t*        fmt_cnt;
};

struct JoinParams {
    const uint32_t* r_codes;
    const uint32_t* r_sweep_start;
    const uint32_t* r_cnt;
    const uint32_t* r_off;
    const uint32_t* surv;
    const uint32_t* surv_cnt;
    const uint32_t* surv_off;
    const uint32_t* item_start;
    const uint32_t* list_start;
    uint64_t        surv_seg_stride;
    uint32_t        nseg, CH, log2NSUB, hash_shift;
    uint32_t        slot;
    uint32_t        bitmap;
    uint64_t*       jsum;
    uint32_t        jobs;
    uint32_t*       nparts;
    uint2*          extra;
    uint32_t*       nextra;
    uint32_t        split_surv;
    uint64_t*       dbg;
    uint32_t        jkind;
    const uint64_t* item_base;
    uint32_t        r_kbits;
    const uint32_t* fmt_cnt;
    uint32_t        timing;
};

struct MatJoinParams {
    const uint32_t* r_codes;
    const uint32_t* r_pay;
    const uint32_t* r_sweep_start;
    const uint32_t* r_cnt;
    const uint32_t* r_off;
    uint32_t        slot;
    const uint32_t* surv;
    const uint32_t* surv_pos;
    const uint32_t* surv_cnt;
    const uint32_t* surv_off;
    const uint32_t* item_start;
    const uint32_t* list_start;
    uint64_t        surv_seg_stride;
    uint32_t        nseg, CH, log2NSUB, hash_shift;
    uint32_t        bm;
    uint32_t        xcd8;
    const uint32_t* s_pay;
    uint2*          out;
    uint64_t        cap;
    unsigned long long* count;
};

void   launch_gen(uint2* out, uint64_t offset, uint64_t count, const GenPlan* d_plan, const Perm& perm,
                  hipStream_t st);
void   launch_zipf(const int32_t* rnd, uint64_t cnt, uint64_t row0, const double* lut,
                   const uint32_t* alphabet, uint32_t size, uint2* out, uint64_t n_above,
                   uint32_t above_base, const Perm& perm, hipStream_t st);
void   launch_build_global(const uint2* R, uint64_t n, const Geometry& g, const CrcTables* tabs,
                           uint32_t* bm, hipStream_t st);
void   launch_probe_global(const uint2* S, uint64_t n, const Geometry& g, const CrcTables* tabs,
                           const uint32_t* bm, uint32_t* out, uint64_t* out_count, hipStream_t st);
void   launch_bitpos(const uint2* R, uint64_t n, const Geometry& g, uint32_t* out, hipStream_t st);
void   launch_slice_fill(const uint32_t* pool, const uint32_t* list, const uint32_t* list_start,
                         const Geometry& g, uint32_t* slices, hipStream_t st);
size_t scatter_lds_bytes(uint32_t log2F);
size_t scatter_pay_lds_bytes(uint32_t log2F);
enum { SIDE_R = 0, SIDE_S = 1 };
void   launch_scatter(const ScatterParams& p, int src, int side, uint32_t grid, hipStream_t st);
void   launch_list_fill(const uint32_t* meta, const uint32_t* wg_used, uint64_t cap,
                        uint32_t log2F, const uint32_t* wgq_off, const uint32_t* colc,
                        const uint64_t* cole, uint32_t CH, uint32_t nseg, uint32_t* list_start,
                        uint64_t* elem_start, uint32_t* item_start, uint32_t* list, uint32_t grid,
                        hipStream_t st);
bool   launch_plan(const uint32_t* wgq_chunks, const uint32_t* wgq_elems, uint32_t G,
                   uint32_t log2F, uint32_t* wgq_off, uint32_t* colc, uint64_t* cole,
                   hipStream_t st);
uint32_t probe_chunks_per_item();
size_t   probe_lds_bytes(const Geometry& g, uint32_t* stage_cap, bool pay = false);
size_t slice_lds_bytes(const Geometry& g);
uint32_t build_chunks_per_sweep();
uint32_t build_sweep_slot();
void   launch_build(const BuildParams& p, uint32_t F, hipStream_t st);
void   launch_probe(const ProbeParams& p, uint32_t grid, hipStream_t st);
size_t probe_bitj_lds_bytes(const Geometry& g);
void   launch_probe_bitj(const ProbeParams& p, uint32_t grid, hipStream_t st);
void   launch_join(const JoinParams& p, uint32_t jobs, uint32_t* job_surv, hipStream_t st);
uint32_t join_extra_tasks();
uint32_t join_sum_slots();
uint32_t join_sum_stride();
uint32_t join_bitmap_log2();
void   launch_join_mat(const MatJoinParams& p, uint32_t jobs, hipStream_t st);
void   launch_mat_build(const uint2* R, uint64_t n, unsigned long long* tab, uint64_t mask,
                        hipStream_t st);
void   launch_mat_probe(const uint2* S, uint64_t n, const uint2* R, const unsigned long long* tab,
                        uint64_t mask, uint2* out, uint64_t cap, unsigned long long* count,
                        const Geometry& g, const uint32_t* slices, const uint32_t* bm,
                        const CrcTables* tabs, hipStream_t st);
void   launch_pj_items(const uint32_t* item_start, const uint32_t* list_start, const uint32_t* cnt,
                       uint32_t items_max, uint32_t F, uint32_t nseg, uint32_t CH, uint64_t seg_words, uint32_t NSUB,
                       uint64_t* region, uint32_t* tot, uint64_t* bsum, uint64_t* sofs, uint64_t* bound,
                       hipStream_t st);
void   launch_pj_recv_scan(const uint32_t* cnt, uint32_t n, uint32_t NSUB, uint32_t* tot, uint64_t* bsum,
                           uint64_t* wscan, hipStream_t st, uint32_t BI = 0, const uint32_t* ritems = nullptr);
void   launch_pj_item_tables(const uint32_t* tab, uint32_t pairs, uint32_t W, const uint32_t* rcnt,
                             const uint64_t* wscan, uint32_t NSUB, uint64_t* ibase, uint32_t* icnt, uint32_t* ioff,
                             uint32_t* jobs, hipStream_t st, uint32_t BI = 0, uint64_t BW = 0);
void   launch_pjx_gather(const uint32_t* pool, const uint32_t* list, const uint32_t* lstart, uint32_t F, uint32_t QL,
                         uint32_t W, uint64_t BR, void* out, uint32_t* ent, int own, void* own_out, uint32_t* own_ent,
                         uint64_t* flag, hipStream_t st);
void   launch_pjx_rtab(const uint64_t* rc, uint32_t W, uint32_t QL, uint32_t NC, uint64_t BR, uint32_t bsw,
                       int64_t* tab, uint32_t* lsO, uint32_t* swO, uint64_t* flag, hipStream_t st);
void   launch_pjx_surv_pack(const uint32_t* surv, const uint64_t* region, const uint32_t* tot, const uint64_t* sofs,
                            const uint32_t* item_start, const uint64_t* bound, const uint32_t* cnt, uint32_t F,
                            uint32_t QL, uint32_t NSUB, uint64_t BI, uint64_t BW, uint32_t* out, uint32_t* out_cnt,
                            int own, uint32_t* own_out, uint32_t* own_cnt, uint64_t* flag, hipStream_t st);
void   launch_pjx_stab(const uint64_t* rc, uint32_t W, uint32_t QL, uint32_t NC, uint64_t BI, uint64_t BW,
                       uint32_t* tab2, uint32_t* istart, uint32_t* ritems, uint64_t* flag, hipStream_t st);
void   launch_pjx_stat(const uint64_t* rc1, const uint64_t* rc2, const uint32_t* ls, const uint32_t* is,
                       const uint64_t* bd, uint32_t W, uint32_t QL, uint32_t NC, const uint64_t* flag, uint64_t* out,
                       hipStream_t st);
struct PjOwn {
    uint32_t  lo = 0, hi = 0;
    int64_t   delta = 0;
    void*     out = nullptr;
    uint32_t* ent = nullptr;
};
void   launch_pj_gather(const uint32_t* pool, const uint32_t* list, uint32_t n, void* out, uint32_t* ent,
                        hipStream_t st, const PjOwn& own = PjOwn{});
void   launch_pj_counts(const uint32_t* starts, const uint64_t* bound, uint32_t W, uint32_t QL, uint32_t NC,
                        uint64_t status, uint64_t extra, uint64_t extra2, uint64_t* out, hipStream_t st);
void   launch_pj_relist(const uint32_t* rent, const int64_t* tab, uint32_t pairs, uint32_t* list,
                        hipStream_t st);
void   launch_pj_surv_pack(const uint32_t* surv, const uint64_t* region, const uint32_t* tot,
                           const uint64_t* soff, uint32_t n, uint32_t* out, hipStream_t st,
                           const PjOwn& own = PjOwn{});
void   launch_export(const uint32_t* slices, const Geometry& g, uint32_t* out, uint64_t nwords,
                     hipStream_t st);
void   launch_copy_bw(const void* src, void* dst, uint64_t bytes, int grid, hipStream_t st);

const char* kernel_build_knobs();

struct DevKnobs {
    bool     kk1 = false;
    bool     kk_gather = false;
    bool     noxcd = false;
    bool     dbg = false;
    uint32_t maxf = 0;
    uint32_t scwpc = 0;
    int      evflags = -1;
    uint32_t l2sub = 0;
    bool     ovl   = false;
    bool     rfirst = false;
};
const DevKnobs& dev_knobs();
std::string dev_knobs_string();

struct TestHooks {
    uint32_t join_split    = 0;
    int      pj_fail_rank  = -1;
    int      bcast_nonroot = 0;
    int      pj_plan_div   = 0;
    int      pj_async_fail = 0;
};
TestHooks& test_hooks();

}
```

### hwbloomradixjoin_amd/csrc/hwbrj_kernels.hip

```cpp
#include <hip/hip_runtime.h>
#include <stdlib.h>

#include <algorithm>
#include <string>
#include <type_traits>

#include "hwbrj_common.h"
#include "hwbrj_kernels.h"

#if !defined(HWBRJ_DEV_BUILD) &&                                                                   \
    (defined(HWBRJ_ABL_NOCRC) || defined(HWBRJ_ABL_NOCRAP) || defined(HWBRJ_ABL_NOSTORE) ||        \
     defined(HWBRJ_ABL_SPLITH) || defined(HWBRJ_ABL_PNOPST) || defined(HWBRJ_ABL_BNOBITS) ||       \
     defined(HWBRJ_ABL_BNOSORT) || defined(HWBRJ_ABL_PNOB1) || defined(HWBRJ_ABL_JNOR) ||          \
     defined(HWBRJ_ABL_JNOS) || defined(HWBRJ_ABL_MJ_EMPTY) || defined(HWBRJ_ABL_MJ_NOLOAD) ||     \
     defined(HWBRJ_ABL_MJ_NOINS) || defined(HWBRJ_ABL_MJ_R) || defined(HWBRJ_ABL_PROBE) ||         \
     defined(HWBRJ_STAMPS))
#error "HWBRJ_ABL_* / HWBRJ_STAMPS give invalid results or perturb timing: dev builds only (-DHWBRJ_DEV_BUILD)"
#endif

namespace hwbrj {

__device__ __forceinline__ void load_tab(uint32_t* dst, const uint32_t* src) {
    for (int i = threadIdx.x; i < 128; i += blockDim.x) dst[i] = src[i];
}
// ... 188 lines not shown
    for (; i < cnt; i += stride) {
        const double r     = ((double) rnd[i]) / 2147483647;
        uint32_t     left  = 0, right = size - 1, pos;
        if (lut[0] >= r) {
            pos = 0;
        } else {
            while (right - left > 1) {
                const uint32_t m = (left + right) / 2;
                if (lut[m] < r) left = m;
                else right = m;
            }
            pos = right;
        }
        const uint64_t row = row0 + i;
        uint32_t       key = alphabet[pos];
        if (n_above) {
            const uint64_t u = perm_apply(perm, row);
            if (u < n_above) key = above_base + (uint32_t) u;
        }
        out[i] = make_uint2(key, (uint32_t) row);
    }
}

void launch_zipf(const int32_t* rnd, uint64_t cnt, uint64_t row0, const double* lut,
                 const uint32_t* alphabet, uint32_t size, uint2* out, uint64_t n_above,
                 uint32_t above_base, const Perm& perm, hipStream_t st) {
    k_zipf<<<8192, 256, 0, st>>>(rnd, cnt, row0, lut, alphabet, size, out, n_above, above_base, perm);
}

__device__ __forceinline__ void global_positions_apply_add(uint32_t key, uint32_t code,
                                                           const Geometry& g, uint32_t* bm) {
    uint64_t base;
    uint32_t size;
    if (g.variant == VAR_BASIC) {
        base = 0;
        size = (uint32_t) g.m;
    } else {
        base = (uint64_t) (code & (g.nblocks - 1u)) * g.block_span;
        size = g.B;
    }
    uint32_t       h  = mod_m(crapwow(kSeed, key), size);
    uint32_t       y  = mod_m(key + kSeed, size);
    const uint32_t s0 = (g.variant == VAR_SECTORIZED) ? h / (g.B < 64u ? g.B : 64u) : 0u;
    for (uint32_t i = 0; i < g.k; i++) {
        const uint32_t pos = (g.variant == VAR_SECTORIZED) ? sectorize(h, s0, i, g.B) : h;
        const uint64_t b   = base + pos;
        atomicOr(bm + (b >> 5), 1u << (uint32_t) (b & 31u));
        h = mod_m(h + y, size);
        y = mod_m(y + i + 1u, size);
    }
}

__device__ __forceinline__ bool global_contains(uint32_t key, uint32_t code, const Geometry& g,
                                                const uint32_t* bm) {
    uint64_t base;
    uint32_t size;
    if (g.variant == VAR_BASIC) {
        base = 0;
        size = (uint32_t) g.m;
    } else {
        base = (uint64_t) (code & (g.nblocks - 1u)) * g.block_span;
        size = g.B;
    }
    uint32_t       h  = mod_m(crapwow(kSeed, key), size);
    uint32_t       y  = mod_m(key + kSeed, size);
    const uint32_t s0 = (g.variant == VAR_SECTORIZED) ? h / (g.B < 64u ? g.B : 64u) : 0u;
    for (uint32_t i = 0; i < g.k; i++) {
        const uint32_t pos = (g.variant == VAR_SECTORIZED) ? sectorize(h, s0, i, g.B) : h;
        const uint64_t b   = base + pos;
        if (!((bm[b >> 5] >> (uint32_t) (b & 31u)) & 1u)) return false;
        h = mod_m(h + y, size);
        y = mod_m(y + i + 1u, size);
    }
    return true;
}

__global__ __launch_bounds__(256) void k_build_global(const uint2* R, uint64_t n, Geometry g,
                                                      const CrcTables* tabs, uint32_t* bm) {
    __shared__ uint32_t fwd[128];
    load_tab(fwd, &tabs->fwd[0][0]);
    __syncthreads();
    uint64_t       i      = blockIdx.x * (uint64_t) blockDim.x + threadIdx.x;
    const uint64_t stride = (uint64_t) gridDim.x * blockDim.x;
    for (; i < n; i += stride) {
        const uint32_t key = R[i].x;
        global_positions_apply_add(key, key_code(fwd, key), g, bm);
    }
}

__global__ __launch_bounds__(1024) void k_probe_global(const uint2* S, uint64_t n, Geometry g,
                                                       const CrcTables* tabs, const uint32_t* bm,
                                                       uint32_t* out, uint64_t* out_count) {
    __shared__ uint32_t fwd[128];
    __shared__ uint32_t wsum[16];
    __shared__ uint64_t bbase;
    load_tab(fwd, &tabs->fwd[0][0]);
    __syncthreads();
    const int wave = threadIdx.x >> 6, lane = threadIdx.x & 63;
    for (uint64_t t0 = (uint64_t) blockIdx.x * 1024; t0 < n; t0 += (uint64_t) gridDim.x * 1024) {
        const uint64_t i    = t0 + threadIdx.x;
        uint32_t       code = 0;
        uint32_t       pass = 0;
        if (i < n) {
            const uint32_t key = S[i].x;
            code               = key_code(fwd, key);
            pass               = global_contains(key, code, g, bm) ? 1u : 0u;
        }
        const uint32_t incl = wave_incl_scan(pass);
        if (lane == 63) wsum[wave] = incl;
        __syncthreads();
        if (threadIdx.x == 0) {
            uint32_t tot = 0;
            for (int w = 0; w < 16; w++) {
                uint32_t c = wsum[w];
                wsum[w]    = tot;
                tot += c;
            }
            bbase = tot ? atomicAdd((unsigned long long*) out_count, (unsigned long long) tot) : 0;
        }
        __syncthreads();
        if (pass) out[bbase + wsum[wave] + incl - 1] = code;
        __syncthreads();
    }
}

__device__ __forceinline__ uint16_t meta16(uint32_t q, uint32_t count) {
    return (uint16_t) (q | ((count - 1u) << 10));
}
#ifndef HWBRJ_SC_T
#define HWBRJ_SC_T 1024
#endif
constexpr int      kScThreads = HWBRJ_SC_T;
constexpr int      kScPlanPer = (1024 + kScThreads - 1) / kScThreads;
constexpr int      kScPayThreads = 1024;
#ifndef HWBRJ_SC_E
#define HWBRJ_SC_E 8
#define HWBRJ_SC_K 2
#endif
#ifndef HWBRJ_SC_PRE
#define HWBRJ_SC_PRE 1
#endif
#ifndef HWBRJ_SC_KEEPY
#define HWBRJ_SC_KEEPY 1
#endif
#ifndef HWBRJ_SC_LAUX
#define HWBRJ_SC_LAUX 2
#endif
#ifndef HWBRJ_SC_SAUX
#define HWBRJ_SC_SAUX 2
#endif
#ifndef HWBRJ_SC_SAUX_R
#define HWBRJ_SC_SAUX_R HWBRJ_SC_SAUX
#endif
constexpr int      kScPre     = HWBRJ_SC_PRE;
constexpr int      kScE       = HWBRJ_SC_E;
constexpr uint32_t kScRound   = kScThreads * kScE;
constexpr int      kScK       = HWBRJ_SC_K;
constexpr uint32_t kCbBits    = 22;
constexpr uint32_t kCbMask    = (1u << kCbBits) - 1u;
constexpr uint32_t kOob       = 0x7FFFFFF0u;

template <int K, bool RIGHT>
__device__ __forceinline__ uint32_t byte_sh2(uint32_t x) {
    static_assert(K >= 0 && K < 4, "byte index");
    uint32_t r;
#define HWBRJ_SDWA(op, sel) asm(op "_sdwa %0, 2, %1 dst_sel:DWORD dst_unused:UNUSED_PAD src0_sel:DWORD src1_sel:" sel : "=v"(r) : "v"(x))
    if (!RIGHT) {
        if (K == 0) HWBRJ_SDWA("v_lshlrev_b32", "BYTE_0");
        if (K == 1) HWBRJ_SDWA("v_lshlrev_b32", "BYTE_1");
        if (K == 2) HWBRJ_SDWA("v_lshlrev_b32", "BYTE_2");
        if (K == 3) HWBRJ_SDWA("v_lshlrev_b32", "BYTE_3");
    } else {
        if (K == 0) HWBRJ_SDWA("v_lshrrev_b32", "BYTE_0");
        if (K == 1) HWBRJ_SDWA("v_lshrrev_b32", "BYTE_1");
        if (K == 2) HWBRJ_SDWA("v_lshrrev_b32", "BYTE_2");
        if (K == 3) HWBRJ_SDWA("v_lshrrev_b32", "BYTE_3");
    }
#undef HWBRJ_SDWA
    return r;
}

__device__ __forceinline__ uint32_t crc_nib(const uint32_t* tab, uint32_t key) {
    const char*    b = (const char*) tab;
    const uint32_t y = key & 0x0F0F0F0Fu, z = key & 0xF0F0F0F0u;
    auto T = [&](uint32_t off) { return *(const uint32_t*) (b + off); };
    const uint32_t t0 = T(byte_sh2<0, false>(y)), t1 = T(byte_sh2<0, true>(z) + 64);
    const uint32_t t2 = T(byte_sh2<1, false>(y) + 128), t3 = T(byte_sh2<1, true>(z) + 192);
    const uint32_t t4 = T(byte_sh2<2, false>(y) + 256), t5 = T(byte_sh2<2, true>(z) + 320);
    const uint32_t t6 = T(byte_sh2<3, false>(y) + 384), t7 = T(byte_sh2<3, true>(z) + 448);
    const uint32_t a = __builtin_amdgcn_bitop3_b32(t0, t1, t2, 0x96);
    const uint32_t c = __builtin_amdgcn_bitop3_b32(t3, t4, t5, 0x96);
    return __builtin_amdgcn_bitop3_b32(a, c, t6 ^ t7, 0x96);
}

template <int SRC, int MODE, int FMT>
__device__ __forceinline__ void sc_word_lds0(uint32_t x, const Geometry& g, const uint32_t* tab,
                                             uint32_t& w, uint32_t& q) {
    const uint32_t F1 = (1u << g.log2F) - 1u;
    if (SRC == SRC_CODES) {
        if (MODE == MODE_BASIC_BITJ) {
            q = basic_bit(bunmix(x), g.bitj, (uint32_t) g.m) & F1;
            w = x;
        } else if (MODE == MODE_CODE_OF_KEY) {
            w = crc_nib(tab, bunmix(x));
            q = w & F1;
        } else {
            w = x;
            q = x & F1;
        }
        return;
    }
    const uint32_t key  = x;
#ifdef HWBRJ_ABL_NOCRC
    const uint32_t code = key * 0x9E3779B1u;
#else
    const uint32_t code = crc_nib(tab, key);
#endif
    if (MODE == MODE_SLICE_BASIC) {
        q = mod_m(crapwow(kSeed, key), (uint32_t) g.m) & F1;
        w = bmix(key);
    } else if (MODE == MODE_SLICE_BLOCK && FMT == FMT_PACKED) {
        q = code & F1;
#ifdef HWBRJ_ABL_NOCRAP
        w = (key & (g.B - 1u)) | ((code >> g.log2F) << g.log2B);
#else
        w = (crapwow(kSeed, key) & (g.B - 1u)) | ((code >> g.log2F) << g.log2B);
#endif
    } else {
        q = code & F1;
        w = code;
    }
}

template <int SRC>
struct ScRaw {
    uint32_t k[SRC == SRC_TUPLES ? kScE : 1];
    uint4    v[SRC == SRC_TUPLES ? 1 : kScE / 4];
    uint32_t jb[SRC == SRC_TUPLES ? kScE : 1];
    uint32_t y[SRC == SRC_TUPLES && HWBRJ_SC_KEEPY ? kScE : 1];
};

template <int SRC, int MODE, int FMT, int SAUX = HWBRJ_SC_SAUX>
__device__ __forceinline__ void scatter_body(const ScatterParams& P) {
    extern __shared__ __attribute__((aligned(16))) uint32_t lds[];
    __shared__ uint32_t crc_tab[128];
    constexpr int NL = SRC == SRC_TUPLES ? kScE / 2 : kScE / 4;
    const uint32_t F     = 1u << P.g.log2F;
    uint32_t*      stage = lds;
    uint32_t*      fill  = stage + F * 32 + 64;
    uint32_t*      ncb   = fill + F + 4;
    uint32_t*      flq   = ncb + 2 * F;
    uint32_t*      misc  = flq + F;
    const int      tid   = threadIdx.x, lane = tid & 63;
    const uint32_t dummy = F * 32 + lane;
    for (uint32_t i = tid; i < F + 1; i += kScThreads) fill[i] = 0;
    uint32_t my_tch[kScPlanPer], my_tel[kScPlanPer];
#pragma unroll
    for (int i = 0; i < kScPlanPer; i++) my_tch[i] = my_tel[i] = 0;
    if (tid < 128) {
        const uint32_t* src = &P.tabs->fwd[0][0];
        uint32_t        v   = src[tid];
        if (tid < 16) {
#pragma unroll
            for (int j = 0; j < 8; j++) v ^= src[j * 16 + ((kSeed >> (4 * j)) & 15u)];
        }
        crc_tab[tid] = v;
    }
    if (tid < 8) misc[tid] = 0;
    if (blockIdx.x == 0 && P.zero_small && tid < 16) P.zero_small[tid] = 0;
    if (blockIdx.x == 0 && P.zero_word && tid == 0) *P.zero_word = 0;

    if (P.dbg && tid == 0) P.dbg[blockIdx.x * 8 + 6] = __builtin_amdgcn_s_memrealtime();
    const uint64_t n     = P.n_dev ? *P.n_dev : P.n;
    const uint64_t units = (n + 3) >> 2;
    const uint64_t G = gridDim.x, wg = blockIdx.x;
    uint64_t       e0  = 4 * (wg * units / G);
    const uint64_t e1r = 4 * ((wg + 1) * units / G);
    const uint64_t e1  = e1r < n ? e1r : n;
    uint32_t       len = __builtin_amdgcn_readfirstlane(e1 > e0 ? (uint32_t) (e1 - e0) : 0u);
    if (SRC == SRC_CODES && P.seg_cnt) {
        e0  = wg * P.seg_stride;
        len = __builtin_amdgcn_readfirstlane(P.seg_cnt[wg]);
    }
    constexpr uint32_t CW = 32u;
    uint32_t* __restrict__ pool = P.pool + wg * P.cap * CW;
    uint16_t* __restrict__ meta = (uint16_t*) P.meta + wg * P.cap;
    constexpr uint32_t EB = SRC == SRC_TUPLES ? 8u : 4u;
    const auto rsrc = buf_rsrc((const uint8_t*) P.src + e0 * EB, len * EB);
    const auto rpool = buf_rsrc(pool, (uint32_t) (P.cap * CW * 4));
    const auto rmeta = buf_rsrc(meta, (uint32_t) (P.cap * 2));
    __syncthreads();

    const uint64_t vn  = MODE == MODE_BASIC_POS && P.vn ? P.vn : 1;
    const uint32_t jb0 = MODE == MODE_BASIC_POS ? (uint32_t) (e0 / vn) : 0u;
    const uint64_t vb  = (uint64_t) (jb0 + 1) * vn;
    auto load_round = [&](uint32_t base, ScRaw<SRC>& R) {
        if (MODE == MODE_BASIC_POS) {
#pragma unroll
            for (int j = 0; j < kScE; j++) {
                const uint32_t i  = base + j * kScThreads + tid;
                const uint64_t ev = e0 + (i < len ? i : 0u);
                uint32_t       jj = jb0;
                for (uint64_t b = vb; ev >= b; b += vn) jj++;
                const uint64_t t = ev - (uint64_t) jj * vn;
                R.k[j]  = len ? ((const uint32_t*) P.src)[2 * t] : 0u;
                R.jb[j] = jj;
            }
        } else if (SRC == SRC_TUPLES && base + kScRound <= len) {
#pragma unroll
            for (int h = 0; h < kScE / 2; h++) {
                const v4u x = __builtin_amdgcn_raw_buffer_load_b128(rsrc, 2 * tid * EB, (base + h * 2 * kScThreads) * EB, HWBRJ_SC_LAUX);
                R.k[2 * h]     = x.x;
                R.k[2 * h + 1] = x.z;
                if (HWBRJ_SC_KEEPY) {
                    R.y[2 * h]     = x.y;
                    R.y[2 * h + 1] = x.w;
                }
            }
        } else if (SRC == SRC_TUPLES) {
#pragma unroll
            for (int j = 0; j < kScE; j++) {
                const uint32_t i = base + (j >> 1) * 2 * kScThreads + 2 * tid + (j & 1);
                R.k[j] = __builtin_amdgcn_raw_buffer_load_b32(rsrc, i < len ? i * EB : kOob, 0, 0);
                if (HWBRJ_SC_KEEPY) R.y[j] = 0;
            }
        } else {
#pragma unroll
            for (int h = 0; h < NL; h++) {
                const uint32_t i = base + h * (4 * kScThreads) + 4 * tid;
                const v4u x = __builtin_amdgcn_raw_buffer_load_b128(rsrc, i < len ? i * EB : kOob, 0, 0);
                R.v[h]      = make_uint4(x.x, x.y, x.z, x.w);
            }
        }
    };
    auto elem = [&](const ScRaw<SRC>& R, uint32_t base, int j, uint32_t& x, uint32_t& idx) {
        if (SRC == SRC_TUPLES) {
            x   = R.k[j];
            idx = MODE == MODE_BASIC_POS ? base + j * kScThreads + tid : base + (j >> 1) * 2 * kScThreads + 2 * tid + (j & 1);
        } else {
            const int h = j >> 2, t = j & 3;
            x   = t == 0 ? R.v[h].x : t == 1 ? R.v[h].y : t == 2 ? R.v[h].z : R.v[h].w;
            idx = base + h * (4 * kScThreads) + 4 * tid + t;
        }
    };
    uint32_t par = 0;
    auto flush_copy = [&]() {
        const uint32_t nf = misc[1 + (par ^ 1u)];
        auto task = [&](uint32_t k) {
            const bool     ok = k < nf * 8;
            const uint32_t qq = flq[ok ? k >> 3 : 0];
            const uint32_t l8 = k & 7;
            const uint32_t cb = ncb[(par ^ 1u) * F + qq] & kCbMask;
            const v4u      v  = *(const v4u*) &stage[qq * 32 + l8 * 4];
#ifdef HWBRJ_ABL_NOSTORE
            if (v.x == 0x12345678u && v.y == 0x9abcdef0u)
#endif
            __builtin_amdgcn_raw_buffer_store_b128(v, rpool, ok ? (cb * 32 + l8 * 4) * 4 : kOob, 0, SAUX);
            __builtin_amdgcn_raw_buffer_store_b16((short) meta16(qq, 32u), rmeta, ok && l8 == 0 ? cb * 2 : kOob, 0, 0);
        };
#pragma unroll
        for (int i = 0; i < kScK; i++) task(tid + i * kScThreads);
        for (uint32_t k = kScK * kScThreads + tid; k < nf * 8; k += kScThreads) task(k);
    };

    uint64_t tph[6] = {0, 0, 0, 0, 0, 0}, tlast = __builtin_amdgcn_s_memtime();
    (void) tlast;
    auto stamp = [&](int k) {
#ifdef HWBRJ_STAMPS
        if (P.dbg) {
            const uint64_t t = __builtin_amdgcn_s_memtime();
            tph[k] += t - tlast;
            tlast = t;
        }
#else
        (void) k;
#endif
    };
    ScRaw<SRC> RA, RB;
    load_round(0, RA);
    if (kScPre == 2) load_round(kScRound, RB);
    constexpr uint32_t kNoPend = 0xFFFFFFFFu;
    uint32_t pq[kScE], pw[kScE];
    bool     pskew = false;
#pragma unroll
    for (int j = 0; j < kScE; j++) pq[j] = kNoPend;
    auto write_pending = [&]() {
        if (!pskew) {
#pragma unroll
            for (int j = 0; j < kScE; j++) stage[pq[j] != kNoPend ? pq[j] - 32u : dummy] = pw[j];
        } else {
#pragma unroll
            for (int j = 0; j < kScE; j++) {
                const bool     ok = pq[j] != kNoPend;
                const uint32_t qq = ok ? pq[j] & 2047u : 0u, sl = pq[j] >> 11;
                const uint32_t cb = ncb[(par ^ 1u) * F + qq], nch = cb >> kCbBits;
                const bool     st = sl >= nch * 32;
                stage[ok && st ? qq * 32 + sl - nch * 32 : dummy] = pw[j];
                const uint32_t po = ((cb & kCbMask) + (sl >> 5)) * 128 + (sl & 31u) * 4;
                __builtin_amdgcn_raw_buffer_store_b32(pw[j], rpool, ok && !st ? po : kOob, 0, 0);
            }
        }
    };

    uint32_t q[kScE], w[kScE];
    auto hash = [&](uint32_t base, const ScRaw<SRC>& R) {
        const bool full = base + kScRound <= len;
        if (SRC == SRC_TUPLES && MODE != MODE_BASIC_POS && HWBRJ_SC_KEEPY) {
#pragma unroll
            for (int j = 0; j < kScE; j++) asm volatile("" ::"v"(R.y[j]));
        }
#pragma unroll
        for (int j = 0; j < kScE; j++) {
            uint32_t x, idx;
            elem(R, base, j, x, idx);
            if (MODE == MODE_BASIC_POS) {
                w[j] = basic_bit(x, R.jb[j], (uint32_t) P.g.m);
                q[j] = w[j] & (F - 1u);
            } else {
                sc_word_lds0<SRC, MODE, FMT>(x, P.g, crc_tab, w[j], q[j]);
            }
            asm volatile("" : "+v"(w[j]));
#ifndef HWBRJ_SC_SB
#define HWBRJ_SC_SB 2
#endif
            if ((j % HWBRJ_SC_SB) == HWBRJ_SC_SB - 1) __builtin_amdgcn_sched_barrier(0);
        }
        if (!full) {
#pragma unroll
            for (int j = 0; j < kScE; j++) {
                uint32_t x, idx;
                elem(R, base, j, x, idx);
                if (idx >= len) q[j] = F;
            }
        }
    };
    auto round = [&](uint32_t base, ScRaw<SRC>& R) {
        const bool full = base + kScRound <= len;
        hash(base, R);
        stamp(0);
        load_round(base + kScPre * kScRound, R);
        uint32_t slot[kScE];
#pragma unroll
        for (int j = 0; j < kScE; j++) slot[j] = atomicAdd(&fill[q[j]], 1u);
        flush_copy();
        if (tid == 0) {
            misc[1 + par]        = 0;
            misc[3 + (par ^ 1u)] = 0;
        }
        stamp(1);
        bool sk = false;
#pragma unroll
        for (int j = 0; j < kScE; j++) {
            q[j] |= slot[j] << 11;
            sk |= q[j] >= (63u << 11) && (q[j] & 2047u) < F;
        }
        if (__builtin_amdgcn_ballot_w64(sk) != 0 && lane == 0) misc[3 + par] = 1u;
        stamp(2);
        __syncthreads();
        stamp(3);
        write_pending();
        const bool skew = __builtin_amdgcn_readfirstlane(misc[3 + par]) != 0;
#pragma unroll
        for (int j = 0; j < kScE; j++) {
            const uint32_t qq = q[j] & 2047u, sl = q[j] >> 11;
            const uint32_t a  = qq * 32 + sl;
            const bool     ok = full || qq < F;
            stage[ok && sl < 32 ? a : dummy] = w[j];
            if (!skew) pq[j] = ok && sl >= 32 ? a : kNoPend;
            else pq[j] = ok && sl >= 32 ? q[j] : kNoPend;
            pw[j] = w[j];
        }
        pskew = skew;
#pragma unroll
        for (int pp = 0; pp < kScPlanPer; pp++) {
            const uint32_t qq  = tid + pp * kScThreads;
            const uint32_t f   = qq < F ? fill[qq] : 0u;
            const uint32_t nch = f >> 5;
            const uint32_t v    = nch | (nch ? (1u << 16) : 0u);
            const uint32_t incl = wave_incl_scan_dpp(v);
            const uint32_t tot  = __builtin_amdgcn_readlane(incl, 63);
            uint32_t       wbc = 0, wbf = 0;
            if (lane == 0 && tot) {
                wbc = atomicAdd(&misc[0], tot & 0xFFFFu);
                wbf = atomicAdd(&misc[1 + par], tot >> 16);
            }
            wbc = __builtin_amdgcn_readfirstlane(wbc);
            wbf = __builtin_amdgcn_readfirstlane(wbf);
            if (nch) {
                const uint32_t cb = wbc + (incl & 0xFFFFu) - nch;
                ncb[par * F + qq] = cb | (nch << kCbBits);
                flq[wbf + (incl >> 16) - 1] = qq;
                fill[qq]          = f & 31u;
                my_tch[pp] += nch;
                my_tel[pp] += nch * 32;
                for (uint32_t c = 1; c < nch; c++) meta[cb + c] = meta16(qq, 32u);
            }
        }
        stamp(4);
        __syncthreads();
        stamp(5);
        par ^= 1u;
    };
    uint32_t base = 0;
    if (kScPre == 2) {
        for (; base + kScRound < len; base += 2 * kScRound) {
            round(base, RA);
            round(base + kScRound, RB);
        }
        if (base < len) round(base, RA);
    } else {
        for (; base < len; base += kScRound) round(base, RA);
    }
    {
        flush_copy();
        __syncthreads();
        write_pending();
        __syncthreads();
#pragma unroll
        for (int pp = 0; pp < kScPlanPer; pp++) {
            const uint32_t qq   = tid + pp * kScThreads;
            const uint32_t f    = qq < F ? fill[qq] : 0u;
            const uint32_t has  = f > 0 ? 1u : 0u;
            const uint32_t incl = wave_incl_scan_dpp(has);
            const uint32_t tot  = __builtin_amdgcn_readlane(incl, 63);
            uint32_t       wb   = 0;
            if (lane == 0 && tot) wb = atomicAdd(&misc[0], tot);
            wb = __builtin_amdgcn_readfirstlane(wb);
            if (has) {
                const uint32_t cb = wb + incl - 1u;
                ncb[qq]  = cb;
                meta[cb] = meta16(qq, f);
                my_tch[pp] += 1;
                my_tel[pp] += f;
            }
        }
        __syncthreads();
        for (uint32_t k = tid; k < F * 8; k += kScThreads) {
            const uint32_t qq = k >> 3, l8 = k & 7;
            const bool     ok = fill[qq] > 0;
            const v4u      v  = *(const v4u*) &stage[qq * 32 + l8 * 4];
            __builtin_amdgcn_raw_buffer_store_b128(v, rpool, ok ? (ncb[qq] * 32 + l8 * 4) * 4 : kOob, 0, 0);
        }
        __syncthreads();
        if (tid == 0) P.wg_used[wg] = misc[0];
        if (P.dbg && tid == 0) {
            for (int k = 0; k < 6; k++) P.dbg[wg * 8 + k] = tph[k];
            P.dbg[wg * 8 + 7] = __builtin_amdgcn_s_memrealtime();
        }
#pragma unroll
        for (int pp = 0; pp < kScPlanPer; pp++) {
            const uint32_t qq = tid + pp * kScThreads;
            if (qq < F) {
                P.wgq_chunks[wg * F + qq] = my_tch[pp];
                P.wgq_elems[wg * F + qq]  = my_tel[pp];
            }
        }
    }
}

constexpr uint32_t kPayDepth = 16;
#ifndef HWBRJ_SC_KP
#define HWBRJ_SC_KP 3
#endif
constexpr int      kScKP     = HWBRJ_SC_KP;
typedef unsigned int v2u __attribute__((ext_vector_type(2)));

template <int MODE, int FMT>
__device__ __forceinline__ void scatter_body_pay(const ScatterParams& P) {
    extern __shared__ __attribute__((aligned(16))) uint32_t lds[];
    __shared__ uint32_t crc_tab[128];
    const uint32_t F     = 1u << P.g.log2F;
    const uint32_t SL    = F * kPayDepth + 64;
    uint2*         stg   = (uint2*) lds;
    uint32_t*      fill  = lds + 2 * SL;
    uint32_t*      pl0   = fill + F + 4;
    uint32_t*      pl1   = pl0 + F;
    uint32_t*      cst   = pl1 + F;
    uint32_t*      tel   = cst + F;
    uint32_t*      flq   = tel + F;
    uint32_t*      misc  = flq + F;
    const int      tid   = threadIdx.x, lane = tid & 63;
    const uint32_t dummy = F * kPayDepth + lane;
    for (uint32_t i = tid; i < F + 1; i += kScPayThreads) fill[i] = 0;
    for (uint32_t i = tid; i < F; i += kScPayThreads) {
        cst[i] = 0;
        tel[i] = 0;
    }
    if (tid < 128) {
        const uint32_t* src = &P.tabs->fwd[0][0];
        uint32_t        v   = src[tid];
        if (tid < 16) {
#pragma unroll
            for (int j = 0; j < 8; j++) v ^= src[j * 16 + ((kSeed >> (4 * j)) & 15u)];
        }
        crc_tab[tid] = v;
    }
    if (tid < 8) misc[tid] = 0;
    if (blockIdx.x == 0 && P.zero_small && tid < 16) P.zero_small[tid] = 0;
    if (blockIdx.x == 0 && P.zero_word && tid == 0) *P.zero_word = 0;

    const uint64_t n     = P.n;
    const uint64_t units = (n + 3) >> 2;
    const uint64_t G = gridDim.x, wg = blockIdx.x;
    const uint64_t e0  = 4 * (wg * units / G);
    const uint64_t e1r = 4 * ((wg + 1) * units / G);
    const uint64_t e1  = e1r < n ? e1r : n;
    const uint32_t len = __builtin_amdgcn_readfirstlane(e1 > e0 ? (uint32_t) (e1 - e0) : 0u);
    uint16_t* __restrict__ meta = (uint16_t*) P.meta + wg * P.cap;
    const auto rsrc   = buf_rsrc((const uint8_t*) P.src + e0 * 8, len * 8);
    const auto rpool  = buf_rsrc(P.pool + wg * P.cap * 32, (uint32_t) (P.cap * 128));
    const auto rppool = buf_rsrc(P.ppool + wg * P.cap * 32, (uint32_t) (P.cap * 128));
    const auto rmeta  = buf_rsrc(meta, (uint32_t) (P.cap * 2));
    __syncthreads();

#ifdef HWBRJ_ABL_SPLITH
    auto hword = [&](uint32_t H) { return (H & 1u) * (uint32_t) (P.cap * 16) + (H >> 1) * 16u; };
#else
    auto hword = [&](uint32_t H) { return H * 16u; };
#endif
    auto load_round = [&](uint32_t base, v2u (&R)[kScE]) {
        if (base + kScRound <= len) {
#pragma unroll
            for (int j = 0; j < kScE; j++)
                R[j] = __builtin_amdgcn_raw_buffer_load_b64(rsrc, tid * 8, (base + j * kScPayThreads) * 8, 0);
        } else {
#pragma unroll
            for (int j = 0; j < kScE; j++) {
                const uint32_t i = base + j * kScPayThreads + tid;
                R[j] = __builtin_amdgcn_raw_buffer_load_b64(rsrc, i < len ? i * 8 : kOob, 0, 0);
            }
        }
    };
    uint32_t par = 0;
    auto flush_copy = [&]() {
        const uint32_t nf = misc[1 + (par ^ 1u)];
        auto task = [&](uint32_t k) {
            const bool     ok = k < nf * 4;
            const uint32_t qq = flq[ok ? k >> 2 : 0];
            const uint32_t l4 = k & 3;
            const uint32_t H  = pl0[qq];
            const v4u      x0 = *(const v4u*) &stg[qq * kPayDepth + l4 * 4];
            const v4u      x1 = *(const v4u*) &stg[qq * kPayDepth + l4 * 4 + 2];
            v4u            vw, vp;
            vw.x = x0.x; vw.y = x0.z; vw.z = x1.x; vw.w = x1.z;
            vp.x = x0.y; vp.y = x0.w; vp.z = x1.y; vp.w = x1.w;
            const uint32_t o  = ok ? (hword(H) + l4 * 4) * 4 : kOob;
            __builtin_amdgcn_raw_buffer_store_b128(vw, rpool, o, 0, 0);
#ifdef HWBRJ_ABL_PNOPST
            if (vp.x == 0x12345678u && vp.y == 0x9abcdef0u)
#endif
            __builtin_amdgcn_raw_buffer_store_b128(vp, rppool, o, 0, 0);
            __builtin_amdgcn_raw_buffer_store_b16((short) meta16(qq, 32u), rmeta, ok && l4 == 0 && (H & 1u) ? (H >> 1) * 2 : kOob, 0, 0);
        };
#pragma unroll
        for (int i = 0; i < kScKP; i++) task(tid + i * kScPayThreads);
        for (uint32_t k = kScKP * kScPayThreads + tid; k < nf * 4; k += kScPayThreads) task(k);
    };
// ... 2577 lines not shown
    pjx_pairs(rc, W, QL, NC, BI, BW, cnt, first, wsum, flag);
    const uint32_t i = threadIdx.x;
    for (uint32_t j = 0; j < W; j++) {
        uint32_t total;
        (void) block_excl_scan(i < QL ? cnt[i * W + j] : 0u, wsum, total);
        if (i == 0) ritems[j] = total;
    }
    uint32_t t = 0;
    if (i < QL)
        for (uint32_t j = 0; j < W; j++) t += cnt[i * W + j];
    uint32_t       total;
    const uint32_t pos = block_excl_scan(i < QL ? t : 0u, wsum, total);
    if (i < QL) {
        istart[i]  = pos;
        uint32_t p = pos;
        for (uint32_t j = 0; j < W; j++) {
            uint32_t* e = tab2 + 3 * ((uint64_t) i * W + j);
            e[0]        = (uint32_t) (j * BI + first[i * W + j]);
            e[1]        = cnt[i * W + j];
            e[2]        = p;
            p += cnt[i * W + j];
        }
    }
    if (i == 0) istart[QL] = total;
}

__global__ __launch_bounds__(1024) void k_pjx_stat(const uint64_t* __restrict__ rc1, const uint64_t* __restrict__ rc2,
                                                   const uint32_t* __restrict__ ls, const uint32_t* __restrict__ is,
                                                   const uint64_t* __restrict__ bd, uint32_t W, uint32_t QL, uint32_t NC,
                                                   const uint64_t* flag, uint64_t* __restrict__ out) {
    __shared__ uint32_t wsum[16];
    const uint32_t i  = threadIdx.x;
    uint64_t       mr = 0, mi = 0, mw = 0;
    for (uint32_t j = 0; j < W; j++) {
        uint32_t r, it;
        (void) block_excl_scan(i < QL ? (uint32_t) rc1[(uint64_t) j * NC + i] : 0u, wsum, r);
        (void) block_excl_scan(i < QL ? (uint32_t) rc2[(uint64_t) j * NC + i] : 0u, wsum, it);
        mr = max(mr, max((uint64_t) r, (uint64_t) (ls[(j + 1) * QL] - ls[j * QL])));
        mi = max(mi, max((uint64_t) it, (uint64_t) (is[(j + 1) * QL] - is[j * QL])));
        mw = max(mw, max(rc2[(uint64_t) j * NC + QL], bd[(j + 1) * QL] - bd[j * QL]));
    }
    if (i == 0) {
        out[0] = *flag;
        out[1] = mr;
        out[2] = mi;
        out[3] = mw;
    }
}

void launch_pjx_gather(const uint32_t* pool, const uint32_t* list, const uint32_t* lstart, uint32_t F, uint32_t QL,
                       uint32_t W, uint64_t BR, void* out, uint32_t* ent, int own, void* own_out, uint32_t* own_ent,
                       uint64_t* flag, hipStream_t st) {
    k_pjx_gather<<<4096, 256, 0, st>>>(pool, list, lstart, F, QL, W, BR, (uint4*) out, ent, own, (uint4*) own_out,
                                       own_ent, flag);
}

void launch_pjx_rtab(const uint64_t* rc, uint32_t W, uint32_t QL, uint32_t NC, uint64_t BR, uint32_t bsw,
                     int64_t* tab, uint32_t* lsO, uint32_t* swO, uint64_t* flag, hipStream_t st) {
    k_pjx_rtab<<<1, 1024, 0, st>>>(rc, W, QL, NC, BR, bsw, tab, lsO, swO, flag);
}

void launch_pjx_surv_pack(const uint32_t* surv, const uint64_t* region, const uint32_t* tot, const uint64_t* sofs,
                          const uint32_t* item_start, const uint64_t* bound, const uint32_t* cnt, uint32_t F,
                          uint32_t QL, uint32_t NSUB, uint64_t BI, uint64_t BW, uint32_t* out, uint32_t* out_cnt,
                          int own, uint32_t* own_out, uint32_t* own_cnt, uint64_t* flag, hipStream_t st) {
    k_pjx_surv_pack<<<2048, 256, 0, st>>>(surv, region, tot, sofs, item_start, bound, cnt, F, QL, NSUB, BI, BW, out,
                                          out_cnt, own, own_out, own_cnt, flag);
}

void launch_pjx_stab(const uint64_t* rc, uint32_t W, uint32_t QL, uint32_t NC, uint64_t BI, uint64_t BW,
                     uint32_t* tab2, uint32_t* istart, uint32_t* ritems, uint64_t* flag, hipStream_t st) {
    k_pjx_stab<<<1, 1024, 0, st>>>(rc, W, QL, NC, BI, BW, tab2, istart, ritems, flag);
}

void launch_pjx_stat(const uint64_t* rc1, const uint64_t* rc2, const uint32_t* ls, const uint32_t* is,
                     const uint64_t* bd, uint32_t W, uint32_t QL, uint32_t NC, const uint64_t* flag, uint64_t* out,
                     hipStream_t st) {
    k_pjx_stat<<<1, 1024, 0, st>>>(rc1, rc2, ls, is, bd, W, QL, NC, flag, out);
}

void launch_gen(uint2* out, uint64_t offset, uint64_t count, const GenPlan* d_plan, const Perm& perm,
                hipStream_t st) {
    k_gen<<<4096, 256, 0, st>>>(out, offset, count, d_plan, perm);
}

void launch_build_global(const uint2* R, uint64_t n, const Geometry& g, const CrcTables* tabs,
                         uint32_t* bm, hipStream_t st) {
    k_build_global<<<4096, 256, 0, st>>>(R, n, g, tabs, bm);
}

void launch_probe_global(const uint2* S, uint64_t n, const Geometry& g, const CrcTables* tabs,
                         const uint32_t* bm, uint32_t* out, uint64_t* out_count, hipStream_t st) {
    k_probe_global<<<2048, 1024, 0, st>>>(S, n, g, tabs, bm, out, out_count);
}

size_t scatter_lds_bytes(uint32_t log2F) {
    const size_t F = 1u << log2F;
    return (F * 32 + 64 + F + 4 + 3 * F + 8) * sizeof(uint32_t);
}

__global__ __launch_bounds__(1024) void k_copy_bw(const uint4* __restrict__ src, uint4* __restrict__ dst, uint64_t n) {
    const uint64_t per = (n + gridDim.x - 1) / gridDim.x;
    const uint64_t b = (uint64_t) blockIdx.x * per, e = min(n, b + per);
    for (uint64_t i = b + threadIdx.x; i < e; i += 4u * 1024u) {
        uint4 v[4];
#pragma unroll
        for (int u = 0; u < 4; u++) {
            const uint64_t k = i + u * 1024u;
            v[u] = k < e ? src[k] : make_uint4(0, 0, 0, 0);
        }
#pragma unroll
        for (int u = 0; u < 4; u++)
            if (i + u * 1024u < e) dst[i + u * 1024u] = v[u];
    }
}

void launch_copy_bw(const void* src, void* dst, uint64_t bytes, int grid, hipStream_t st) {
    k_copy_bw<<<grid, 1024, 0, st>>>((const uint4*) src, (uint4*) dst, bytes / 16);
}

template <int SRC, int MODE, int FMT>
__global__ __launch_bounds__(kScThreads) void k_scatter_r(ScatterParams P) { scatter_body<SRC, MODE, FMT, HWBRJ_SC_SAUX_R>(P); }
template <int SRC, int MODE, int FMT>
__global__ __launch_bounds__(kScThreads) void k_scatter_s(ScatterParams P) { scatter_body<SRC, MODE, FMT>(P); }

template <int SRC, int MODE, int FMT>
static void scatter_inst(const ScatterParams& p, int side, uint32_t grid, hipStream_t st) {
    const size_t lds = scatter_lds_bytes(p.g.log2F);
    const void*  fn  = side == SIDE_R ? (const void*) &k_scatter_r<SRC, MODE, FMT> : (const void*) &k_scatter_s<SRC, MODE, FMT>;
    (void) hipFuncSetAttribute(fn, hipFuncAttributeMaxDynamicSharedMemorySize, (int) lds);
    if (side == SIDE_R) k_scatter_r<SRC, MODE, FMT><<<grid, kScThreads, lds, st>>>(p);
    else k_scatter_s<SRC, MODE, FMT><<<grid, kScThreads, lds, st>>>(p);
}

size_t scatter_pay_lds_bytes(uint32_t log2F) {
    const size_t F = (size_t) 1 << log2F;
    return (2 * (F * kPayDepth + 64) + F + 4 + 5 * F + 8) * sizeof(uint32_t);
}

template <int MODE, int FMT>
__global__ __launch_bounds__(kScPayThreads) void k_scatter_rp(ScatterParams P) { scatter_body_pay<MODE, FMT>(P); }
template <int MODE, int FMT>
__global__ __launch_bounds__(kScPayThreads) void k_scatter_sp(ScatterParams P) { scatter_body_pay<MODE, FMT>(P); }

template <int MODE, int FMT>
static void scatter_pay_inst(const ScatterParams& p, int side, uint32_t grid, hipStream_t st) {
    const size_t lds = scatter_pay_lds_bytes(p.g.log2F);
    const void*  fn  = side == SIDE_R ? (const void*) &k_scatter_rp<MODE, FMT> : (const void*) &k_scatter_sp<MODE, FMT>;
    (void) hipFuncSetAttribute(fn, hipFuncAttributeMaxDynamicSharedMemorySize, (int) lds);
    if (side == SIDE_R) k_scatter_rp<MODE, FMT><<<grid, kScPayThreads, lds, st>>>(p);
    else k_scatter_sp<MODE, FMT><<<grid, kScPayThreads, lds, st>>>(p);
}

void launch_scatter(const ScatterParams& p, int src, int side, uint32_t grid, hipStream_t st) {
    const Geometry& g = p.g;
    if (p.ppool) {
        switch (g.mode) {
            case MODE_SLICE_BLOCK:
                if (g.format == FMT_PACKED) return scatter_pay_inst<MODE_SLICE_BLOCK, FMT_PACKED>(p, side, grid, st);
                return scatter_pay_inst<MODE_SLICE_BLOCK, FMT_CODE>(p, side, grid, st);
            case MODE_SLICE_BASIC: return scatter_pay_inst<MODE_SLICE_BASIC, FMT_CODE>(p, side, grid, st);
            default: return scatter_pay_inst<MODE_NOBLOOM, FMT_CODE>(p, side, grid, st);
        }
    }
    if (src == SRC_CODES) {
        if (g.mode == MODE_BASIC_BITJ) return scatter_inst<SRC_CODES, MODE_BASIC_BITJ, FMT_CODE>(p, side, grid, st);
        if (g.mode == MODE_CODE_OF_KEY) return scatter_inst<SRC_CODES, MODE_CODE_OF_KEY, FMT_CODE>(p, side, grid, st);
        return scatter_inst<SRC_CODES, MODE_GLOBAL, FMT_CODE>(p, side, grid, st);
    }
    switch (g.mode) {
        case MODE_SLICE_BLOCK:
            if (g.format == FMT_PACKED)
                return scatter_inst<SRC_TUPLES, MODE_SLICE_BLOCK, FMT_PACKED>(p, side, grid, st);
            return scatter_inst<SRC_TUPLES, MODE_SLICE_BLOCK, FMT_CODE>(p, side, grid, st);
        case MODE_SLICE_BASIC:
            return scatter_inst<SRC_TUPLES, MODE_SLICE_BASIC, FMT_CODE>(p, side, grid, st);
        case MODE_BASIC_POS: return scatter_inst<SRC_TUPLES, MODE_BASIC_POS, FMT_CODE>(p, side, grid, st);
        default: return scatter_inst<SRC_TUPLES, MODE_NOBLOOM, FMT_CODE>(p, side, grid, st);
    }
}

void launch_list_fill(const uint32_t* meta, const uint32_t* wg_used, uint64_t cap, uint32_t log2F,
                      const uint32_t* wgq_off, const uint32_t* colc, const uint64_t* cole,
                      uint32_t CH, uint32_t nseg, uint32_t* list_start, uint64_t* elem_start,
                      uint32_t* item_start, uint32_t* list, uint32_t grid, hipStream_t st) {
    const size_t lds = (kLfBatch + 4 * (1u << log2F) + 16) * sizeof(uint32_t);
    (void) hipFuncSetAttribute((const void*) &k_list_fill, hipFuncAttributeMaxDynamicSharedMemorySize, (int) lds);
    k_list_fill<<<grid, kLfThreads, lds, st>>>(meta, wg_used, cap, log2F, wgq_off, colc, cole, CH,
                                               nseg, list_start, elem_start, item_start, list);
}

bool launch_plan(const uint32_t* wgq_chunks, const uint32_t* wgq_elems, uint32_t G, uint32_t log2F,
                 uint32_t* wgq_off, uint32_t* colc, uint64_t* cole, hipStream_t st) {
    if (G > kPlanRGs * kPlanMaxRG) return false;
    const uint32_t F = 1u << log2F;
    k_plan<<<(F + kPlanCols - 1) / kPlanCols, 1024, 0, st>>>(wgq_chunks, wgq_elems, G, log2F, wgq_off, colc, cole);
    return true;
}

size_t slice_lds_bytes(const Geometry& g) {
    const bool slices = g.mode == MODE_SLICE_BLOCK || g.mode == MODE_SLICE_BASIC;
    return ((slices ? g.seg_words : 0) + 128 + kBSlot + 128) * sizeof(uint32_t);
}

uint32_t build_chunks_per_sweep() { return kBSweep; }
uint32_t build_sweep_slot() { return kBSlot; }

int consumer_kind(const Geometry& g) {
    if (g.mode == MODE_SLICE_BASIC) return g.k == 1 ? KIND_BASIC_K1 : KIND_BASIC_KK;
    if (g.mode == MODE_SLICE_BLOCK)
        return g.format == FMT_PACKED ? (g.k == 1 ? KIND_BLOCK_PK1 : KIND_BLOCK_PKK) : KIND_BLOCK;
    return KIND_PASS;
}


template <int KIND>
static void build_inst(const BuildParams& p, uint32_t F, size_t lds, hipStream_t st) {
    if (p.ppool) {
        (void) hipFuncSetAttribute((const void*) &k_build<KIND, true>, hipFuncAttributeMaxDynamicSharedMemorySize, (int) lds);
        k_build<KIND, true><<<F, 1024, lds, st>>>(p);
        return;
    }
    (void) hipFuncSetAttribute((const void*) &k_build<KIND>, hipFuncAttributeMaxDynamicSharedMemorySize, (int) lds);
    k_build<KIND><<<F, 1024, lds, st>>>(p);
}

template <int KIND>
static void probe_inst(const ProbeParams& p, uint32_t grid, size_t lds, hipStream_t st) {
    if (p.surv_pos) {
        if (KIND == KIND_PASS || p.g.nseg == 1) {
            (void) hipFuncSetAttribute((const void*) &k_probe<KIND, true, true>, hipFuncAttributeMaxDynamicSharedMemorySize, (int) lds);
            k_probe<KIND, true, true><<<grid, 1024, lds, st>>>(p);
        } else {
            (void) hipFuncSetAttribute((const void*) &k_probe<KIND, false, true>, hipFuncAttributeMaxDynamicSharedMemorySize, (int) lds);
            k_probe<KIND, false, true><<<grid, 1024, lds, st>>>(p);
        }
        return;
    }
    if (KIND == KIND_PASS || p.g.nseg == 1) {
        (void) hipFuncSetAttribute((const void*) &k_probe<KIND, true>, hipFuncAttributeMaxDynamicSharedMemorySize, (int) lds);
        k_probe<KIND, true><<<grid, 1024, lds, st>>>(p);
    } else {
        (void) hipFuncSetAttribute((const void*) &k_probe<KIND, false>, hipFuncAttributeMaxDynamicSharedMemorySize, (int) lds);
        k_probe<KIND, false><<<grid, 1024, lds, st>>>(p);
    }
}

void launch_build(const BuildParams& p, uint32_t F, hipStream_t st) {
    const size_t lds = slice_lds_bytes(p.g);
    switch (consumer_kind(p.g)) {
        case KIND_BLOCK_PK1: return build_inst<KIND_BLOCK_PK1>(p, F, lds, st);
        case KIND_BLOCK_PKK: return build_inst<KIND_BLOCK_PKK>(p, F, lds, st);
        case KIND_BLOCK: return build_inst<KIND_BLOCK>(p, F, lds, st);
        case KIND_BASIC_K1: return build_inst<KIND_BASIC_K1>(p, F, lds, st);
        case KIND_BASIC_KK: return build_inst<KIND_PASS>(p, F, lds, st);
        default: return build_inst<KIND_PASS>(p, F, lds, st);
    }
}

size_t probe_lds_bytes(const Geometry& g, uint32_t* stage_cap, bool pay) {
    const bool   slices = g.mode == MODE_SLICE_BLOCK || g.mode == MODE_SLICE_BASIC;
    const size_t NSUB   = (size_t) 1 << g.log2NSUB;
    const int    kind   = consumer_kind(g);
    const size_t scap   = pay ? 0 : kind == KIND_BLOCK_PKK || kind == KIND_BASIC_KK
                              ? scr_cap<KIND_BLOCK_PKK>() : scr_cap<KIND_PASS>();
    const size_t base   = ((slices ? g.seg_words : 0) + 3 * 128 + 16 * NSUB + 16 * scap + 64) * sizeof(uint32_t);
    size_t cap = std::min<size_t>(kProbeCH * 32, (163840 - 512 - base) / 8 - 64) & ~(size_t) 7;
    if (!pay) cap = std::min<size_t>(cap, (size_t) (slices ? kPco : kPC) * 4096);
    if (stage_cap) *stage_cap = (uint32_t) cap;
    return base + 2 * (cap + 64) * 4;
}

void launch_probe(const ProbeParams& p0, uint32_t grid, hipStream_t st) {
    ProbeParams p = p0;
    const size_t lds = probe_lds_bytes(p.g, &p.stage_cap, p.surv_pos != nullptr);
    switch (consumer_kind(p.g)) {
        case KIND_BLOCK_PK1: return probe_inst<KIND_BLOCK_PK1>(p, grid, lds, st);
        case KIND_BLOCK_PKK: return probe_inst<KIND_BLOCK_PKK>(p, grid, lds, st);
        case KIND_BLOCK: return probe_inst<KIND_BLOCK>(p, grid, lds, st);
        case KIND_BASIC_K1: return probe_inst<KIND_BASIC_K1>(p, grid, lds, st);
        case KIND_BASIC_KK: return probe_inst<KIND_BASIC_KK>(p, grid, lds, st);
        default: return probe_inst<KIND_PASS>(p, grid, lds, st);
    }
}

uint32_t probe_chunks_per_item() { return kProbeCH; }

void launch_join(const JoinParams& p0, uint32_t jobs, uint32_t* job_surv, hipStream_t st) {
    JoinParams p = p0;
    p.jobs       = jobs;
    const uint32_t split = p.split_surv ? p.split_surv : kJoinTaskSurv;
    k_join_split<<<(jobs + 255) / 256, 256, 0, st>>>(p.item_start, job_surv, p.log2NSUB, jobs, split,
                                                     p.nparts, p.extra, p.nextra, p.jsum);
    if (p.r_kbits == 18) k_join<18><<<jobs + kJoinExtra, kJoinThreads, 0, st>>>(p);
    else if (p.r_kbits == 24) k_join<24><<<jobs + kJoinExtra, kJoinThreads, 0, st>>>(p);
    else k_join<32><<<jobs + kJoinExtra, kJoinThreads, 0, st>>>(p);
    k_join_mixed<<<std::min<uint32_t>(jobs + kJoinExtra, 1024u), kJoinThreads, 0, st>>>(p);
}

uint32_t join_extra_tasks() { return kJoinExtra; }
uint32_t join_sum_slots() { return kJoinSumSlots; }
uint32_t join_sum_stride() { return kJoinSumStride; }
uint32_t join_bitmap_log2() { return kJoinBmLog2; }

void launch_export(const uint32_t* slices, const Geometry& g, uint32_t* out, uint64_t nwords,
                   hipStream_t st) {
    k_export<<<2048, 256, 0, st>>>(slices, g, out, nwords);
}

const char* kernel_build_knobs() {
    static const std::string s = [] {
        std::string r;
        auto num = [&](const char* n, long v, long d) {
            if (v != d) r += std::string(r.empty() ? "" : " ") + n + "=" + std::to_string(v);
        };
        auto flag = [&](const char* n) { r += std::string(r.empty() ? "" : " ") + n; };
        (void) flag;
#ifdef HWBRJ_DEV_BUILD
        flag("HWBRJ_DEV_BUILD");
#endif
        num("HWBRJ_SC_T", HWBRJ_SC_T, 1024);
        num("HWBRJ_SC_E", HWBRJ_SC_E, 8);
        num("HWBRJ_SC_K", HWBRJ_SC_K, 2);
        num("HWBRJ_SC_PRE", HWBRJ_SC_PRE, 1);
        num("HWBRJ_SC_KEEPY", HWBRJ_SC_KEEPY, 1);
        num("HWBRJ_SC_LAUX", HWBRJ_SC_LAUX, 2);
        num("HWBRJ_SC_SAUX", HWBRJ_SC_SAUX, 2);
        num("HWBRJ_SC_SAUX_R", HWBRJ_SC_SAUX_R, 2);
        num("HWBRJ_SC_SB", HWBRJ_SC_SB, 2);
        num("HWBRJ_SC_KP", HWBRJ_SC_KP, 3);
        num("HWBRJ_PLANCOLS", HWBRJ_PLANCOLS, 16);
        num("HWBRJ_LFPER", HWBRJ_LFPER, 28);
        num("HWBRJ_BPQ", HWBRJ_BPQ, 2);
        num("HWBRJ_BD_NT", HWBRJ_BD_NT, 0);
        num("HWBRJ_PC", HWBRJ_PC, 3);
        num("HWBRJ_SCR1", HWBRJ_SCR1, 128);
        num("HWBRJ_PR_NT", HWBRJ_PR_NT, 0);
        num("HWBRJ_SCRK", HWBRJ_SCRK, 256);
        num("HWBRJ_JTU", HWBRJ_JTU, 8);
        num("HWBRJ_JTS", HWBRJ_JTS, 2);
        num("HWBRJ_JT", HWBRJ_JT, 256);
        num("HWBRJ_JXCD", HWBRJ_JXCD, 1);
        num("HWBRJ_PACK3", HWBRJ_PACK3, 1);
        num("HWBRJ_PACK18", HWBRJ_PACK18, 1);
        num("HWBRJ_JRR", HWBRJ_JRR, 4);
        num("HWBRJ_JRW", HWBRJ_JRW, 4);
        num("HWBRJ_JSR", HWBRJ_JSR, 8);
        num("HWBRJ_JFS", HWBRJ_JFS, 5);
        num("HWBRJ_JSW", HWBRJ_JSW, 2);
        num("HWBRJ_JFR", HWBRJ_JFR, 8);
        num("HWBRJ_JFW", HWBRJ_JFW, 5);
        num("HWBRJ_JBM", HWBRJ_JBM, 18);
        num("HWBRJ_OVL_ASYNC", HWBRJ_OVL_ASYNC, 1);
        num("HWBRJ_PJ_OVL", HWBRJ_PJ_OVL, 1);
        num("HWBRJ_ABL_PROBE", HWBRJ_ABL_PROBE, 0);
        num("HWBRJ_PCO", HWBRJ_PCO, 1);
        num("HWBRJ_PCO_AUX", HWBRJ_PCO_AUX, 0);
#define HWBRJ_FLAG_KNOB(X) flag(#X)
#ifdef HWBRJ_STAMPS
        HWBRJ_FLAG_KNOB(HWBRJ_STAMPS);
#endif
#ifdef HWBRJ_ABL_NOCRC
        HWBRJ_FLAG_KNOB(HWBRJ_ABL_NOCRC);
#endif
#ifdef HWBRJ_ABL_NOCRAP
        HWBRJ_FLAG_KNOB(HWBRJ_ABL_NOCRAP);
#endif
#ifdef HWBRJ_ABL_NOSTORE
        HWBRJ_FLAG_KNOB(HWBRJ_ABL_NOSTORE);
#endif
#ifdef HWBRJ_ABL_SPLITH
        HWBRJ_FLAG_KNOB(HWBRJ_ABL_SPLITH);
#endif
#ifdef HWBRJ_ABL_PNOPST
        HWBRJ_FLAG_KNOB(HWBRJ_ABL_PNOPST);
#endif
#ifdef HWBRJ_ABL_BNOBITS
        HWBRJ_FLAG_KNOB(HWBRJ_ABL_BNOBITS);
#endif
#ifdef HWBRJ_ABL_BNOSORT
        HWBRJ_FLAG_KNOB(HWBRJ_ABL_BNOSORT);
#endif
#ifdef HWBRJ_ABL_PNOB1
        HWBRJ_FLAG_KNOB(HWBRJ_ABL_PNOB1);
#endif
#ifdef HWBRJ_ABL_JNOR
        HWBRJ_FLAG_KNOB(HWBRJ_ABL_JNOR);
#endif
#ifdef HWBRJ_ABL_JNOS
        HWBRJ_FLAG_KNOB(HWBRJ_ABL_JNOS);
#endif
#ifdef HWBRJ_ABL_MJ_EMPTY
        HWBRJ_FLAG_KNOB(HWBRJ_ABL_MJ_EMPTY);
#endif
#ifdef HWBRJ_ABL_MJ_NOLOAD
        HWBRJ_FLAG_KNOB(HWBRJ_ABL_MJ_NOLOAD);
#endif
#ifdef HWBRJ_ABL_MJ_NOINS
        HWBRJ_FLAG_KNOB(HWBRJ_ABL_MJ_NOINS);
#endif
#ifdef HWBRJ_ABL_MJ_R
        HWBRJ_FLAG_KNOB(HWBRJ_ABL_MJ_R);
#endif
#undef HWBRJ_FLAG_KNOB
        return r;
    }();
    return s.c_str();
}

}
```

### include/hwbrj.h

```cpp
#ifndef HWBRJ_H
#define HWBRJ_H

#include <stdint.h>

#ifdef __cplusplus
extern "C" {
#endif

#ifdef KEY_8B
#error "libhwbrj joins 8-byte tuples (src/types.h without KEY_8B); KEY_8B is not supported"
#endif
#ifndef TYPES_H
#define TYPES_H
typedef int32_t intkey_t;
typedef int32_t value_t;

typedef struct tuple_t    tuple_t;
typedef struct relation_t relation_t;
typedef struct result_t       result_t;
typedef struct threadresult_t threadresult_t;

struct tuple_t {
    intkey_t key;
    value_t  payload;
// ... 22 lines not shown

typedef struct bloom_filter_args_t {
    bloom_filter_variant_t variant;
    uint64_t               m;
    uint64_t               k;
    uint64_t               B;
} bloom_filter_args_t;

void assert_args(bloom_filter_args_t * args);
#endif
#define HWBRJ_SECTORIZED ((bloom_filter_variant_t) 2)

result_t * BPRO(relation_t * relR, relation_t * relS, int nthreads,
                bloom_filter_args_t * bloom_filter_args);
result_t * PRO(relation_t * relR, relation_t * relS, int nthreads);
result_t * BPRH(relation_t * relR, relation_t * relS, int nthreads,
                bloom_filter_args_t * bloom_filter_args);
result_t * BPRHO(relation_t * relR, relation_t * relS, int nthreads,
                 bloom_filter_args_t * bloom_filter_args);
result_t * BRJ(relation_t * relR, relation_t * relS, int nthreads,
               bloom_filter_args_t * bloom_filter_args);
result_t * PRH(relation_t * relR, relation_t * relS, int nthreads);
result_t * PRHO(relation_t * relR, relation_t * relS, int nthreads);
result_t * RJ(relation_t * relR, relation_t * relS, int nthreads);
result_t * hwbrj_BPRO(relation_t * relR, relation_t * relS, int nthreads,
                      bloom_filter_args_t * bloom_filter_args);
result_t * hwbrj_PRO(relation_t * relR, relation_t * relS, int nthreads);

typedef struct hwbrj_stats_t {
    uint64_t filtered;
    int64_t  matches;
    int      mode;
    int      format;
    uint32_t partitions;
    uint32_t subparts;
    uint32_t slice_segments;
    double   ms_total;
    double   ms_r_scatter;
    double   ms_r_index;
    double   ms_build;
    double   ms_s_scatter;
    double   ms_s_index;
    double   ms_probe;
    double   ms_surv;
    double   ms_join;
    double   ms_join_probe;
    int      join_keys;
    uint32_t unstaged_items;
    uint32_t join_key_bits;
} hwbrj_stats_t;
enum { HWBRJ_JOIN_KEYS_32 = 0, HWBRJ_JOIN_KEYS_PACKED = 1, HWBRJ_JOIN_KEYS_MIXED = 2 };

int hwbrj_join_device(const tuple_t * d_R, uint64_t nR, const tuple_t * d_S, uint64_t nS,
                      const bloom_filter_args_t * args, void * stream, hwbrj_stats_t * stats);
enum { HWBRJ_ALGO_PRO = 0, HWBRJ_ALGO_PRH = 1, HWBRJ_ALGO_PRHO = 2 };
int hwbrj_join_device_algo(const tuple_t * d_R, uint64_t nR, const tuple_t * d_S, uint64_t nS,
                           const bloom_filter_args_t * args, int algorithm, void * stream,
                           hwbrj_stats_t * stats);
int hwbrj_join_device_async(const tuple_t * d_R, uint64_t nR, const tuple_t * d_S, uint64_t nS,
                            const bloom_filter_args_t * args, void * stream);
int hwbrj_join_wait(hwbrj_stats_t * stats);
int hwbrj_join_wait_all(hwbrj_stats_t * stats, int capacity, int * n_joins);
int hwbrj_set_async_timing(int on);

int hwbrj_join_materialize_device(const tuple_t * d_R, uint64_t nR, const tuple_t * d_S,
                                  uint64_t nS, const bloom_filter_args_t * args, tuple_t * d_out,
                                  uint64_t capacity, uint64_t * n_out, void * stream,
                                  hwbrj_stats_t * stats, double * ms_materialize);
void hwbrj_set_materialize(int on);
int  hwbrj_set_gpus(int gpus);

typedef enum {
    HWBRJ_PJ_R_SEND = 0, HWBRJ_PJ_R_SEND_ENT, HWBRJ_PJ_R_RECV, HWBRJ_PJ_R_RECV_ENT,
    HWBRJ_PJ_SLICES, HWBRJ_PJ_S_SEND, HWBRJ_PJ_S_RECV, HWBRJ_PJ_M_SEND, HWBRJ_PJ_M_RECV,
    HWBRJ_PJ_NSLOTS
} hwbrj_pj_slot_t;

typedef struct hwbrj_exchange_t {
    void * ctx;
    void * (*buffer)(void * ctx, int slot, uint64_t bytes);
    int (*alltoall_u64)(void * ctx, const uint64_t * send, uint64_t * recv, uint64_t n);
    int (*alltoallv)(void * ctx, int send_slot, const uint64_t * soff, const uint64_t * sbytes,
                     int recv_slot, const uint64_t * roff, const uint64_t * rbytes);
    int (*allgather)(void * ctx, int slot, uint64_t bytes);
} hwbrj_exchange_t;

int hwbrj_join_partitioned(const hwbrj_exchange_t * x, int rank, int world, const tuple_t * d_R,
                           uint64_t nR, uint64_t nR_total, const tuple_t * d_S, uint64_t nS,
                           const bloom_filter_args_t * args, hwbrj_stats_t * stats);

int hwbrj_comm_unique_id(uint8_t * unique_id_out );
int hwbrj_comm_init(const uint8_t * unique_id , int world, int rank);
int hwbrj_comm_destroy(void);
int hwbrj_comm_info(int * world, int * rank);
int hwbrj_set_filter_broadcast(int on);
int hwbrj_join_partitioned_rccl(const tuple_t * d_R, uint64_t nR, uint64_t nR_total,
                                const tuple_t * d_S, uint64_t nS, const bloom_filter_args_t * args,
                                hwbrj_stats_t * stats);
int hwbrj_join_partitioned_rccl_async(const tuple_t * d_R, uint64_t nR, uint64_t nR_total,
                                      const tuple_t * d_S, uint64_t nS,
                                      const bloom_filter_args_t * args);
int hwbrj_join_partitioned_async(const hwbrj_exchange_t * x, int rank, int world, const tuple_t * d_R,
                                 uint64_t nR, uint64_t nR_total, const tuple_t * d_S, uint64_t nS,
                                 const bloom_filter_args_t * args);
int hwbrj_join_partitioned_wait(hwbrj_stats_t * stats);
int hwbrj_pj_async_info(uint64_t * out );

int hwbrj_generate_device(tuple_t * d_out, uint64_t n, uint32_t nthreads, uint64_t maxid,
                          uint64_t threshold, double selectivity, uint64_t seed, void * stream);
int hwbrj_generate_device_range(tuple_t * d_out, uint64_t n, uint64_t offset, uint64_t count,
                                uint32_t nthreads, uint64_t maxid, uint64_t threshold,
                                double selectivity, uint64_t seed, void * stream);
int hwbrj_generate_host(tuple_t * out, uint64_t n, uint32_t nthreads, uint64_t maxid,
                        uint64_t threshold, double selectivity, uint64_t seed, int host_threads);

uint64_t hwbrj_nonunique_threshold(uint64_t r_size, double selectivity, int full_range);
int      hwbrj_create_relation_nonunique(tuple_t * out, uint64_t n, int64_t maxid, uint32_t seed);
int      hwbrj_create_relation_nonunique_from_pk(tuple_t * out, uint64_t n, const tuple_t * pk,
                                                 uint64_t npk, int64_t threshold,
                                                 double selectivity, uint32_t seed);
int      hwbrj_create_relation_fk_from_pk(tuple_t * out, uint64_t n, const tuple_t * pk,
                                          uint64_t npk, int64_t threshold, double selectivity,
                                          uint32_t seed);
int      hwbrj_create_relation_zipf(tuple_t * out, uint64_t n, uint64_t alphabet_size,
                                    double theta, uint32_t seed, int host_threads);
int      hwbrj_create_relation_zipf_device(tuple_t * d_out, uint64_t n, uint64_t alphabet_size,
                                           double theta, uint32_t seed, double selectivity,
                                           int host_threads, void * stream);
int      hwbrj_rand_stream(uint32_t seed, int32_t * out, uint64_t n);

int hwbrj_write_relation(const relation_t * rel, const char * filename);
int hwbrj_write_result_relation(const result_t * res, const char * filename);

int hwbrj_export_filter(uint8_t * host_out, uint64_t nbytes);

uint64_t hwbrj_tsc_hz(void);

int hwbrj_copy_bandwidth(uint64_t bytes, int reps, double * gbps);

uint32_t hwbrj_hash_crc(uint32_t seed, int32_t key);
uint32_t hwbrj_hash_crapwow(uint32_t seed, int32_t key);

int          hwbrj_device_count(void);
int          hwbrj_set_device(int device);
void         hwbrj_release(void);
const char * hwbrj_last_error(void);
const char * hwbrj_version(void);

enum {
    HWBRJ_HOOK_JOIN_SPLIT     = 1,
    HWBRJ_HOOK_PJ_FAIL_RANK   = 2,
    HWBRJ_HOOK_BCAST_NONROOT  = 3,
    HWBRJ_HOOK_PJ_PLAN_DIV    = 4,
    HWBRJ_HOOK_PJ_ASYNC_FAIL  = 5
};
int          hwbrj_set_test_hook(int hook, int64_t value);

#ifdef __cplusplus
}
#endif
#endif
```

Baseline: 248.4 billion.

## Add work-stealing tail pool to the radix scatter kernel

The scatter kernel now gives each workgroup a fixed number of static rounds and places the remaining tail (about 1/16 of rounds) in a shared pool. Workgroups claim pool rounds with atomic tickets fetched one round ahead, so uneven workgroup progress does not leave stragglers at the end of the scatter. Per-workgroup region capacity is sized for static plus maximum stolen rounds, and double-buffered counters are reset between launches. This adds atomic traffic and extra per-round control logic, and it requires a single round of prefetch.

New measurement: 248.3 billion (median of 2 runs). No clear change (-0.0%).

```diff
diff --git a/hwbloomradixjoin_amd/__init__.py b/hwbloomradixjoin_amd/__init__.py
--- a/hwbloomradixjoin_amd/__init__.py
+++ b/hwbloomradixjoin_amd/__init__.py
@@ -158,6 +158,9 @@
         L.hwbrj_version.restype = ctypes.c_char_p
         L.hwbrj_set_test_hook.restype = ctypes.c_int
         L.hwbrj_set_test_hook.argtypes = [ctypes.c_int, ctypes.c_int64]
+        L.hwbrj_scatter_split.restype = ctypes.c_int
+        L.hwbrj_scatter_split.argtypes = [ctypes.c_uint64, ctypes.c_uint32, ctypes.c_uint32,
+                                          ctypes.POINTER(ctypes.c_uint64)]
         L.hwbrj_tsc_hz.restype = ctypes.c_uint64
         L.hwbrj_copy_bandwidth.restype = ctypes.c_int
         L.hwbrj_copy_bandwidth.argtypes = [ctypes.c_uint64, ctypes.c_int, ctypes.POINTER(ctypes.c_double)]
@@ -250,8 +253,9 @@
 
 
 HOOK_JOIN_SPLIT, HOOK_PJ_FAIL_RANK, HOOK_BCAST_NONROOT, HOOK_PJ_PLAN_DIV, HOOK_PJ_ASYNC_FAIL = 1, 2, 3, 4, 5
+HOOK_SC_STEAL_ALL = 6
 _HOOK_OFF = {HOOK_JOIN_SPLIT: 0, HOOK_PJ_FAIL_RANK: -1, HOOK_BCAST_NONROOT: 0, HOOK_PJ_PLAN_DIV: 0,
-             HOOK_PJ_ASYNC_FAIL: 0}
+             HOOK_PJ_ASYNC_FAIL: 0, HOOK_SC_STEAL_ALL: 0}
 
 
 def version() -> str:
@@ -269,6 +273,12 @@
         yield
     finally:
         set_test_hook(hook, _HOOK_OFF[hook])
+
+
+def scatter_split(n: int, G: int, F: int = 1024) -> tuple:
+    out = (ctypes.c_uint64 * 4)()
+    _err(lib().hwbrj_scatter_split(int(n), int(G), int(F), out), "hwbrj_scatter_split")
+    return tuple(int(x) for x in out)
 
 
 def set_gpus(gpus: int) -> None:
diff --git a/hwbloomradixjoin_amd/csrc/hwbrj_api.cpp b/hwbloomradixjoin_amd/csrc/hwbrj_api.cpp
--- a/hwbloomradixjoin_amd/csrc/hwbrj_api.cpp
+++ b/hwbloomradixjoin_amd/csrc/hwbrj_api.cpp
@@ -46,6 +46,7 @@
     if (h.bcast_nonroot) add("HWBRJ_HOOK_BCAST_NONROOT=" + std::to_string(h.bcast_nonroot));
     if (h.pj_plan_div) add("HWBRJ_HOOK_PJ_PLAN_DIV=" + std::to_string(h.pj_plan_div));
     if (h.pj_async_fail) add("HWBRJ_HOOK_PJ_ASYNC_FAIL=" + std::to_string(h.pj_async_fail));
+    if (h.sc_steal_all) add("HWBRJ_HOOK_SC_STEAL_ALL=" + std::to_string(h.sc_steal_all));
     const std::string v = std::string("hwbloomradixjoin_amd 0.6 (gfx950) src " HWBRJ_SRC_SHA) +
                           (k.empty() ? "" : " knobs: " + k);
     return interned.insert(v).first->c_str();
@@ -73,12 +74,29 @@
             if (value < 0 || value > 1) break;
             h.pj_async_fail = (int) value;
             return 0;
+        case HWBRJ_HOOK_SC_STEAL_ALL:
+            if (value < 0 || value > 1) break;
+            h.sc_steal_all = (int) value;
+            return 0;
         default:
             set_last_error("unknown test hook");
             return 2;
     }
     set_last_error("test hook value out of range");
     return 2;
+}
+
+int hwbrj_scatter_split(uint64_t n, uint32_t G, uint32_t F, uint64_t out[4]) {
+    if (!out || G == 0 || G > 512 || F == 0 || F > 1024) {
+        set_last_error("hwbrj_scatter_split: G in [1, 512], F in [1, 1024]");
+        return 2;
+    }
+    const ScatterSplit s = scatter_split(n, G, F, test_hooks().sc_steal_all != 0);
+    out[0] = s.static_rounds;
+    out[1] = s.pool_rounds;
+    out[2] = s.steal_max;
+    out[3] = s.cap;
+    return 0;
 }
 
 int hwbrj_device_count(void) {
diff --git a/hwbloomradixjoin_amd/csrc/hwbrj_engine.cpp b/hwbloomradixjoin_amd/csrc/hwbrj_engine.cpp
--- a/hwbloomradixjoin_amd/csrc/hwbrj_engine.cpp
+++ b/hwbloomradixjoin_amd/csrc/hwbrj_engine.cpp
@@ -289,7 +289,7 @@
                       &istartS, &listS, &slices, &bitmap, &rjoin, &rrun, &surv, &survcnt, &survoff,
                       &dense, &small, &bpos, &colR, &colS, &mtab, &mcount, &jtask, &jparts, &pjList,
                       &pjLstart, &pjSweep, &pjTab, &pjRegion, &pjTot, &pjSoff, &pjIbase, &pjCnt, &pjOff,
-                      &pjIstart, &pjJobs, &ppoolR, &ppoolS, &rpay, &survpos, &dense2, &kkcnt, &xcnt_, &pjBsum, &pjBound, &pjWtot, &pjWscan, &pjTab2})
+                      &pjIstart, &pjJobs, &ppoolR, &ppoolS, &rpay, &survpos, &dense2, &kkcnt, &xcnt_, &pjBsum, &pjBound, &pjWtot, &pjWscan, &pjTab2, &stealcnt})
         b->release();
     for (DevBuf& b : xslot_) b.release();
     if (pending_) (void) hipEventSynchronize(ev_[8]);
@@ -300,11 +300,7 @@
 
 static size_t ring_slot_bytes() { return 128 + join_sum_slots() * join_sum_stride() * 8; }
 
-static uint64_t region_cap(uint64_t n, uint32_t G, uint32_t F) {
-    const uint64_t units = (n + 3) / 4;
-    const uint64_t per   = ((units + G - 1) / G) * 4;
-    return (per + 31) / 32 + F + 1;
-}
+static uint64_t region_cap(uint64_t n, uint32_t G, uint32_t F) { return scatter_static_cap(n, G, F); }
 
 int Engine::run(const uint2* dR, uint64_t nR, const uint2* dS, uint64_t nS,
                 const bloom_filter_args_t* args, hipStream_t stream, hwbrj_stats_t* st, int jkind) {
@@ -315,7 +311,7 @@
 int Engine::run_async(const uint2* dR, uint64_t nR, const uint2* dS, uint64_t nS,
                       const bloom_filter_args_t* args, hipStream_t stream, int jkind) {
     phase_ev_    = false;
-    const int rc = enqueue(dR, nR, dS, nS, args, stream, false, jkind);
+    const int rc = enqueue(dR, nR, dS, nS, args, stream, dev_knobs().dbg, jkind);
     phase_ev_    = true;
     return rc;
 }
@@ -383,7 +379,11 @@
         if (!bcast || alloc_only_) return rc;
         return rccl_agree_status(comm_, comm_world_, comm_rank_, rc, stream, &agree_);
     };
-    const uint64_t capR = region_cap(nR, G, F), capS = region_cap(std::max(nS, nRk), G, F);
+    const bool         all_pool = test_hooks().sc_steal_all != 0;
+    const ScatterSplit splR = scatter_split(nR, G, F, all_pool), splS = scatter_split(nS, G, F, all_pool);
+    const bool         stealR = splR.steal && !mat, stealS = splS.steal && !mat && g.mode != MODE_GLOBAL;
+    const uint64_t capR = stealR ? splR.cap : region_cap(nR, G, F);
+    const uint64_t capS = std::max(stealS ? splS.cap : region_cap(nS, G, F), region_cap(nRk, G, F));
     const uint64_t LR = (uint64_t) G * capR, LS = (uint64_t) G * capS;
     const uint64_t items_max = (LS / CH + F + 1) * nseg;
     if (G > 512) {
@@ -415,6 +415,12 @@
     const bool jnew = jparts.bytes < (size_t) (2 * NJ + 1) * 4 || NJ != last_nj_;
     last_nj_ = NJ;
     ok &= jtask.ensure((size_t) join_extra_tasks() * 8) && jparts.ensure((size_t) (2 * NJ + 1) * 4);
+    if (!stealcnt.p && stealcnt.ensure(64)) {
+        ok &= hipMemset(stealcnt.p, 0, stealcnt.bytes) == hipSuccess && hipDeviceSynchronize() == hipSuccess;
+        steal_par_[0] = steal_par_[1] = 0;
+        steal_clean_[0] = steal_clean_[1] = true;
+    }
+    ok &= stealcnt.p != nullptr;
     if (slice_mode) ok &= slices.ensure((uint64_t) F * nseg * g.seg_words * 4);
     if (g.mode == MODE_GLOBAL) ok &= bitmap.ensure(((g.m + 31) / 32) * 4) && dense.ensure(nS * 4);
     if (basic_kk) ok &= bpos.ensure(nRk * 4);
@@ -444,6 +450,22 @@
     sp.g    = g;
     sp.zero_small = (uint32_t*) sm;
     sp.zero_word  = jparts.as<uint32_t>() + 2 * NJ;
+    auto steal_set = [&](ScatterParams& p, int side, const ScatterSplit& sl, hipStream_t st) -> hipError_t {
+        uint32_t* w     = stealcnt.as<uint32_t>() + 2 * side;
+        p.steal         = w + steal_par_[side];
+        p.steal_next    = w + (steal_par_[side] ^ 1u);
+        p.static_rounds = (uint32_t) sl.static_rounds;
+        p.pool_rounds   = (uint32_t) sl.pool_rounds;
+        p.steal_max     = (uint32_t) sl.steal_max;
+        const hipError_t e = steal_clean_[side] ? hipSuccess : hipMemsetAsync(p.steal, 0, 4, st);
+        steal_clean_[side] = false;
+        return e;
+    };
+    auto steal_done = [&](int side) {
+        if (hipPeekAtLastError() != hipSuccess) return;
+        steal_clean_[side] = true;
+        steal_par_[side] ^= 1u;
+    };
 
     auto s_pass = [&](hipStream_t st, bool marks, hipEvent_t* tev = nullptr) -> int {
         ScatterParams ss = sp;
@@ -475,8 +497,10 @@
             ss.dbg = dbgS.as<uint64_t>();
         }
         ss.ppool = mat ? ppoolS.as<uint32_t>() : nullptr;
+        if (stealS) HWBRJ_CHECK(steal_set(ss, SIDE_S, splS, st));
         if (tev) HWBRJ_CHECK(hipEventRecord(tev[0], st));
         launch_scatter(ss, g.mode == MODE_GLOBAL ? SRC_CODES : SRC_TUPLES, SIDE_S, G, st);
+        if (stealS) steal_done(SIDE_S);
         if (tev) HWBRJ_CHECK(hipEventRecord(tev[1], st));
         if (marks) HWBRJ_CHECK(mark(4, st));
         launch_plan(wgqcS.as<uint32_t>(), wgqeS.as<uint32_t>(), G, g.log2F, wgqoS.as<uint32_t>(),
@@ -523,7 +547,19 @@
     sp.wgq_chunks = wgqcR.as<uint32_t>();
     sp.wgq_elems  = wgqeR.as<uint32_t>();
     sp.cap        = capR;
+    if (dbg) {
+        if (!dbgR.ensure((size_t) G * 64)) {
+            set_last_error("hipMalloc failed (device memory)");
+            return 4;
+        }
+        HWBRJ_CHECK(hipMemsetAsync(dbgR.p, 0, dbgR.bytes, stream));
+        sp.dbg = dbgR.as<uint64_t>();
+    }
+    if (stealR) HWBRJ_CHECK(steal_set(sp, SIDE_R, splR, stream));
     launch_scatter(sp, SRC_TUPLES, SIDE_R, G, stream);
+    if (stealR) steal_done(SIDE_R);
+    sp.steal = sp.steal_next = nullptr;
+    sp.dbg = nullptr;
     HWBRJ_CHECK(mark(1, stream));
     launch_plan(wgqcR.as<uint32_t>(), wgqeR.as<uint32_t>(), G, g.log2F, wgqoR.as<uint32_t>(),
                 colR.as<uint32_t>() + 2 * F, colR.as<uint64_t>(), stream);
@@ -720,19 +756,23 @@
             for (int k = 0; k < 6; k++) ss[k] += (double) hs[b * 8 + k] / G;
         fprintf(stderr, "[dbg] S scatter cyc/WG: hash %.0f load+flush %.0f rank %.0f b1 %.0f write+plan %.0f b2 %.0f\n",
                 ss[0], ss[1], ss[2], ss[3], ss[4], ss[5]);
-        {
-            uint64_t t0 = ~0ull;
+        std::vector<uint64_t> hr(G * 8);
+        HWBRJ_CHECK(hipMemcpy(hr.data(), dbgR.p, hr.size() * 8, hipMemcpyDeviceToHost));
+        uint64_t t0 = ~0ull;
+        for (uint32_t b = 0; b < G; b++) t0 = std::min<uint64_t>(t0, std::min(hs[b * 8 + 6], hr[b * 8 + 6]));
+        auto spread = [&](const char* name, const std::vector<uint64_t>& h) {
             std::vector<double> st(G), en(G);
-            for (uint32_t b = 0; b < G; b++) t0 = std::min<uint64_t>(t0, hs[b * 8 + 6]);
             for (uint32_t b = 0; b < G; b++) {
-                st[b] = (hs[b * 8 + 6] - t0) / 100.0;
-                en[b] = (hs[b * 8 + 7] - t0) / 100.0;
+                st[b] = (h[b * 8 + 6] - t0) / 100.0;
+                en[b] = (h[b * 8 + 7] - t0) / 100.0;
             }
             std::sort(st.begin(), st.end());
             std::sort(en.begin(), en.end());
-            fprintf(stderr, "[dbg] S scatter WG start us: max %.1f | end us: min %.1f p10 %.1f p50 %.1f p90 %.1f max %.1f\n",
-                    st[G - 1], en[0], en[G / 10], en[G / 2], en[G * 9 / 10], en[G - 1]);
-        }
+            fprintf(stderr, "[dbg] %s scatter WG start us: min %.1f p50 %.1f max %.1f | end us: min %.1f p10 %.1f p50 %.1f p90 %.1f max %.1f\n",
+                    name, st[0], st[G / 2], st[G - 1], en[0], en[G / 10], en[G / 2], en[G * 9 / 10], en[G - 1]);
+        };
+        spread("R", hr);
+        spread("S", hs);
         fprintf(stderr, "[dbg] probe cyc/WG: top %.0f test %.0f b1 %.0f scan+b2 %.0f write %.0f b3+copy %.0f\n",
                 sp_[0], sp_[1], sp_[2], sp_[3], sp_[4], sp_[5]);
         {
diff --git a/hwbloomradixjoin_amd/csrc/hwbrj_engine.h b/hwbloomradixjoin_amd/csrc/hwbrj_engine.h
--- a/hwbloomradixjoin_amd/csrc/hwbrj_engine.h
+++ b/hwbloomradixjoin_amd/csrc/hwbrj_engine.h
@@ -194,13 +194,16 @@
     GenPlan*     d_plan_ = nullptr;
     DevBuf poolR, metaR, usedR, wgqcR, wgqeR, wgqoR, lstartR, estartR, istartR, listR;
     DevBuf poolS, metaS, usedS, wgqcS, wgqeS, wgqoS, lstartS, estartS, istartS, listS;
-    DevBuf slices, bitmap, rjoin, rrun, surv, survcnt, survoff, dense, small, dbgP, dbgJ, dbgS;
+    DevBuf slices, bitmap, rjoin, rrun, surv, survcnt, survoff, dense, small, dbgP, dbgJ, dbgS, dbgR;
     DevBuf bpos;
     DevBuf colR, colS;
     DevBuf mtab, mcount;
     DevBuf ppoolR, ppoolS, rpay, survpos;
     DevBuf dense2, kkcnt;
     DevBuf jtask, jparts;
+    DevBuf   stealcnt;
+    uint32_t steal_par_[2]   = {0, 0};
+    bool     steal_clean_[2] = {true, true};
     DevBuf pjList, pjLstart, pjSweep, pjTab, pjRegion, pjTot, pjSoff, pjIbase, pjCnt, pjOff, pjIstart, pjJobs;
     DevBuf pjBsum, pjBound, pjWtot, pjWscan, pjTab2;
 };
diff --git a/hwbloomradixjoin_amd/csrc/hwbrj_kernels.h b/hwbloomradixjoin_amd/csrc/hwbrj_kernels.h
--- a/hwbloomradixjoin_amd/csrc/hwbrj_kernels.h
+++ b/hwbloomradixjoin_amd/csrc/hwbrj_kernels.h
@@ -29,6 +29,11 @@
     uint64_t         vn;
     uint32_t*        zero_small;
     uint32_t*        zero_word;
+    uint32_t*        steal;
+    uint32_t*        steal_next;
+    uint32_t         static_rounds;
+    uint32_t         pool_rounds;
+    uint32_t         steal_max;
     Geometry         g;
     const CrcTables* tabs;
 };
@@ -159,6 +164,12 @@
 size_t scatter_pay_lds_bytes(uint32_t log2F);
 enum { SIDE_R = 0, SIDE_S = 1 };
 void   launch_scatter(const ScatterParams& p, int src, int side, uint32_t grid, hipStream_t st);
+struct ScatterSplit {
+    uint64_t static_rounds, pool_rounds, steal_max, cap;
+    bool     steal;
+};
+ScatterSplit scatter_split(uint64_t n, uint32_t G, uint32_t F, bool all_pool = false);
+uint64_t     scatter_static_cap(uint64_t n, uint32_t G, uint32_t F);
 void   launch_list_fill(const uint32_t* meta, const uint32_t* wg_used, uint64_t cap,
                         uint32_t log2F, const uint32_t* wgq_off, const uint32_t* colc,
                         const uint64_t* cole, uint32_t CH, uint32_t nseg, uint32_t* list_start,
@@ -253,6 +264,7 @@
     int      bcast_nonroot = 0;
     int      pj_plan_div   = 0;
     int      pj_async_fail = 0;
+    int      sc_steal_all  = 0;
 };
 TestHooks& test_hooks();
 
diff --git a/hwbloomradixjoin_amd/csrc/hwbrj_kernels.hip b/hwbloomradixjoin_amd/csrc/hwbrj_kernels.hip
--- a/hwbloomradixjoin_amd/csrc/hwbrj_kernels.hip
+++ b/hwbloomradixjoin_amd/csrc/hwbrj_kernels.hip
@@ -364,6 +364,10 @@
 #ifndef HWBRJ_SC_SAUX_R
 #define HWBRJ_SC_SAUX_R HWBRJ_SC_SAUX
 #endif
+#ifndef HWBRJ_SC_STEAL
+#define HWBRJ_SC_STEAL 16
+#endif
+static_assert(HWBRJ_SC_STEAL == 0 || HWBRJ_SC_PRE == 1, "the stolen tail fetches its tickets for one round of loads in flight");
 constexpr int      kScPre     = HWBRJ_SC_PRE;
 constexpr int      kScE       = HWBRJ_SC_E;
 constexpr uint32_t kScRound   = kScThreads * kScE;
@@ -478,9 +482,26 @@
         }
         crc_tab[tid] = v;
     }
-    if (tid < 8) misc[tid] = 0;
+    if (tid < 5) misc[tid] = 0;
     if (blockIdx.x == 0 && P.zero_small && tid < 16) P.zero_small[tid] = 0;
     if (blockIdx.x == 0 && P.zero_word && tid == 0) *P.zero_word = 0;
+    constexpr bool     ST        = SRC == SRC_TUPLES && MODE != MODE_BASIC_POS && HWBRJ_SC_STEAL != 0;
+    constexpr uint32_t kNoTicket = 0xFFFFFFFFu;
+    const bool         steal     = ST && P.steal != nullptr;
+    auto ticket = [&](bool elig) {
+        const auto rc = buf_rsrc(P.steal, elig ? 4u : 0u);
+        return (uint32_t) __builtin_amdgcn_raw_ptr_buffer_atomic_add_i32(1, rc, tid * 4, 0, 0);
+    };
+    if (steal) {
+        if (blockIdx.x == 0 && tid == 0) *P.steal_next = 0;
+        const bool     k0 = P.static_rounds == 0 && P.steal_max > 0;
+        const bool     k1 = P.static_rounds <= 1 && 1u - P.static_rounds < P.steal_max;
+        const uint32_t t0 = ticket(k0), t1 = ticket(k1);
+        if (tid == 0) {
+            misc[5] = k0 ? t0 : kNoTicket;
+            misc[6] = k1 ? t1 : kNoTicket;
+        }
+    }
 
     if (P.dbg && tid == 0) P.dbg[blockIdx.x * 8 + 6] = __builtin_amdgcn_s_memrealtime();
     const uint64_t n     = P.n_dev ? *P.n_dev : P.n;
@@ -494,6 +515,11 @@
         e0  = wg * P.seg_stride;
         len = __builtin_amdgcn_readfirstlane(P.seg_cnt[wg]);
     }
+    if (steal) {
+        e0  = wg * P.static_rounds * kScRound;
+        len = P.static_rounds * kScRound;
+    }
+    const uint64_t pool_e0 = G * P.static_rounds * kScRound;
     constexpr uint32_t CW = 32u;
     uint32_t* __restrict__ pool = P.pool + wg * P.cap * CW;
     uint16_t* __restrict__ meta = (uint16_t*) P.meta + wg * P.cap;
@@ -506,7 +532,7 @@
     const uint64_t vn  = MODE == MODE_BASIC_POS && P.vn ? P.vn : 1;
     const uint32_t jb0 = MODE == MODE_BASIC_POS ? (uint32_t) (e0 / vn) : 0u;
     const uint64_t vb  = (uint64_t) (jb0 + 1) * vn;
-    auto load_round = [&](uint32_t base, ScRaw<SRC>& R) {
+    auto load_round = [&](__amdgpu_buffer_rsrc_t rsrc, uint32_t len, uint32_t base, ScRaw<SRC>& R) {
         if (MODE == MODE_BASIC_POS) {
 #pragma unroll
             for (int j = 0; j < kScE; j++) {
@@ -588,9 +614,29 @@
         (void) k;
 #endif
     };
+    uint32_t rno = 0, cur_cnt = 0;
+    auto round_at = [&](uint32_t r, uint32_t tslot, uint64_t& start, uint32_t& cnt) {
+        const uint64_t off = (uint64_t) r * kScRound;
+        start = e0 + off;
+        cnt   = 0;
+        if (off < len) {
+            cnt = len - (uint32_t) off < kScRound ? len - (uint32_t) off : kScRound;
+        } else if (steal) {
+            const uint32_t t = __builtin_amdgcn_readfirstlane(misc[5 + tslot]);
+            start = pool_e0 + (uint64_t) (t < P.pool_rounds ? t : 0u) * kScRound;
+            if (t < P.pool_rounds) cnt = n - start < kScRound ? (uint32_t) (n - start) : kScRound;
+        }
+    };
+    auto round_rsrc = [&](uint64_t start, uint32_t cnt) { return buf_rsrc((const uint8_t*) P.src + start * EB, cnt * EB); };
     ScRaw<SRC> RA, RB;
-    load_round(0, RA);
-    if (kScPre == 2) load_round(kScRound, RB);
+    if (ST) {
+        uint64_t s0;
+        round_at(0, 0, s0, cur_cnt);
+        load_round(round_rsrc(s0, cur_cnt), cur_cnt, 0, RA);
+    } else {
+        load_round(rsrc, len, 0, RA);
+        if (kScPre == 2) load_round(rsrc, len, kScRound, RB);
+    }
     constexpr uint32_t kNoPend = 0xFFFFFFFFu;
     uint32_t pq[kScE], pw[kScE];
     bool     pskew = false;
@@ -615,7 +661,7 @@
     };
 
     uint32_t q[kScE], w[kScE];
-    auto hash = [&](uint32_t base, const ScRaw<SRC>& R) {
+    auto hash = [&](uint32_t len, uint32_t base, const ScRaw<SRC>& R) {
         const bool full = base + kScRound <= len;
         if (SRC == SRC_TUPLES && MODE != MODE_BASIC_POS && HWBRJ_SC_KEEPY) {
 #pragma unroll
@@ -647,10 +693,22 @@
         }
     };
     auto round = [&](uint32_t base, ScRaw<SRC>& R) {
-        const bool full = base + kScRound <= len;
-        hash(base, R);
+        const uint32_t rlen = ST ? cur_cnt : len;
+        const bool     full = base + kScRound <= rlen;
+        hash(rlen, base, R);
         stamp(0);
-        load_round(base + kScPre * kScRound, R);
+        uint32_t nxt_cnt = 0, tk = 0;
+        bool     tk_ok   = false;
+        if (ST) {
+            uint64_t ns;
+            round_at(rno + 1, par ^ 1u, ns, nxt_cnt);
+            const uint32_t sr = P.static_rounds;
+            tk_ok = steal && nxt_cnt != 0 && rno + 2 >= sr && rno + 2 - sr < P.steal_max;
+            tk    = ticket(tk_ok);
+            load_round(round_rsrc(ns, nxt_cnt), nxt_cnt, 0, R);
+        } else {
+            load_round(rsrc, len, base + kScPre * kScRound, R);
+        }
         uint32_t slot[kScE];
 #pragma unroll
         for (int j = 0; j < kScE; j++) slot[j] = atomicAdd(&fill[q[j]], 1u);
@@ -708,13 +766,20 @@
                 for (uint32_t c = 1; c < nch; c++) meta[cb + c] = meta16(qq, 32u);
             }
         }
+        if (ST && steal && tid == 0) misc[5 + par] = tk_ok ? tk : kNoTicket;
         stamp(4);
         __syncthreads();
         stamp(5);
         par ^= 1u;
+        if (ST) {
+            cur_cnt = nxt_cnt;
+            rno++;
+        }
     };
     uint32_t base = 0;
-    if (kScPre == 2) {
+    if (ST) {
+        while (cur_cnt) round(0, RA);
+    } else if (kScPre == 2) {
         for (; base + kScRound < len; base += 2 * kScRound) {
             round(base, RA);
             round(base + kScRound, RB);
@@ -3598,6 +3663,28 @@
     else k_scatter_sp<MODE, FMT><<<grid, kScPayThreads, lds, st>>>(p);
 }
 
+uint64_t scatter_static_cap(uint64_t n, uint32_t G, uint32_t F) {
+    const uint64_t units = (n + 3) / 4;
+    const uint64_t per   = ((units + G - 1) / G) * 4;
+    return (per + 31) / 32 + F + 1;
+}
+
+ScatterSplit scatter_split(uint64_t n, uint32_t G, uint32_t F, bool all_pool) {
+    ScatterSplit s{};
+    if (HWBRJ_SC_STEAL == 0 || G == 0) {
+        s.cap = scatter_static_cap(n, G ? G : 1, F);
+        return s;
+    }
+    const uint64_t rounds = n / kScRound + (n % kScRound ? 1 : 0);
+    const uint64_t pool = all_pool ? rounds : std::max<uint64_t>(rounds / HWBRJ_SC_STEAL, rounds ? 1 : 0);
+    s.static_rounds = (rounds - pool) / G;
+    s.pool_rounds   = rounds - s.static_rounds * G;
+    s.steal_max     = (2 * s.pool_rounds + G - 1) / G;
+    s.cap           = ((s.static_rounds + s.steal_max) * kScRound + 31) / 32 + F + 1;
+    s.steal         = true;
+    return s;
+}
+
 void launch_scatter(const ScatterParams& p, int src, int side, uint32_t grid, hipStream_t st) {
     const Geometry& g = p.g;
     if (p.ppool) {
@@ -3775,6 +3862,7 @@
         num("HWBRJ_SC_SAUX_R", HWBRJ_SC_SAUX_R, 2);
         num("HWBRJ_SC_SB", HWBRJ_SC_SB, 2);
         num("HWBRJ_SC_KP", HWBRJ_SC_KP, 3);
+        num("HWBRJ_SC_STEAL", HWBRJ_SC_STEAL, 16);
         num("HWBRJ_PLANCOLS", HWBRJ_PLANCOLS, 16);
         num("HWBRJ_LFPER", HWBRJ_LFPER, 28);
         num("HWBRJ_BPQ", HWBRJ_BPQ, 2);
diff --git a/include/hwbrj.h b/include/hwbrj.h
--- a/include/hwbrj.h
+++ b/include/hwbrj.h
@@ -198,9 +198,12 @@
     HWBRJ_HOOK_PJ_FAIL_RANK   = 2,
     HWBRJ_HOOK_BCAST_NONROOT  = 3,
     HWBRJ_HOOK_PJ_PLAN_DIV    = 4,
-    HWBRJ_HOOK_PJ_ASYNC_FAIL  = 5
+    HWBRJ_HOOK_PJ_ASYNC_FAIL  = 5,
+    HWBRJ_HOOK_SC_STEAL_ALL   = 6
 };
 int          hwbrj_set_test_hook(int hook, int64_t value);
+
+int          hwbrj_scatter_split(uint64_t n, uint32_t G, uint32_t F, uint64_t out[4]);
 
 #ifdef __cplusplus
 }
```
